# lucidrains/x-clip

Measured on AMD Instinct MI355X. Metric: image-text pairs/sec (fwd+bwd) at global batch; MFMA% + HBM GB/s, higher is better.
Workload: dtype bf16; 1 GPU; BASELINE configs[1]: default CLIP dim 512 depth 6/6 image 256 patch 32 text seq 256, patch dropout 0.5, InfoNCE, fwd+bwd; the last text layer computes only the CLS row the head reads (the same loss and gradients up to bf16 rounding order; the dense layer is timed in `dense_last_layer` with --full); workload_tag=default-infonce-b1024, local_batch=1024, global_batch=1024, parallelism=dp1, text_last_layer_rows=cls-only

## Files before the change

include/xclip.h:

```cpp
#ifndef XCLIP_H
#define XCLIP_H
#include <stdint.h>

#ifdef __cplusplus
extern "C" {
#endif

enum { XCLIP_F32 = 0, XCLIP_BF16 = 1 };
#define XCLIP_ABI_VERSION 28

int xclip_abi_version(void);
const char* xclip_last_error(void);
const char* xclip_build_info(void);
int xclip_clock_sample(uint64_t* out2, int64_t ticks_10ns, void* stream);

int xclip_layernorm_fwd(const void* x, int64_t ldx, const void* g, const void* res, void* y, int64_t ldy, int64_t y_grp,
                        float* mean, float* rstd, int64_t rows, int64_t dim, float eps, int geglu, int dtype, void* stream);
int64_t xclip_layernorm_bwd_workspace_bytes(int64_t rows, int64_t dim);
int xclip_layernorm_bwd(const void* dy, const void* x, int64_t ldx, const void* g, const float* mean, const float* rstd,
                        const void* dres, void* dx, int64_t lddx, float* dg_accum, void* workspace, int64_t workspace_bytes,
                        int64_t rows, int64_t dim, int geglu, int dtype, void* stream);

int xclip_layernorm_chain_fwd(const void* p, const void* g1, const void* res, void* x1, float* mean1, float* rstd1, const void* g2,
                              void* h2, float* mean2, float* rstd2, int64_t rows, int64_t dim, float eps, int dtype, void* stream);
int64_t xclip_layernorm_chain_bwd_workspace_bytes(int64_t rows, int64_t dim);
int xclip_layernorm_chain_bwd(const void* dh2, const void* x1, const void* g2, const float* mean2, const float* rstd2, const void* dres,
                              void* dx1, const void* p, const void* g1, const float* mean1, const float* rstd1, void* dp, float* dg2_accum,
                              float* dg1_accum, void* workspace, int64_t workspace_bytes, int64_t rows, int64_t dim, int dtype, void* stream);
int xclip_l2norm_fwd(const void* x, void* y, float* rnorm, int64_t rows, int64_t dim, int dtype, void* stream);
int xclip_l2norm_bwd(const void* dy, const void* y, const float* rnorm, void* dx, int64_t rows, int64_t dim, int dtype, void* stream);

int xclip_text_embed_fwd(const int64_t* tokens, const void* E, const void* P, const void* cls, void* out,
                         int64_t batch, int64_t n, int64_t dim, int64_t vocab, int32_t* bad_token_flag, int dtype, void* stream);
int xclip_text_embed_bwd(const void* dout, const int64_t* tokens, float* dE_accum, float* dP_accum, float* dcls_accum,
                         int64_t batch, int64_t n, int64_t dim, int64_t vocab, int has_cls, int dtype, void* stream);

int xclip_patchify(const void* image, const int32_t* keep, void* out, int64_t ldo, int64_t batch, int64_t channels,
                   int64_t height, int64_t width, int64_t patch, int64_t nkeep, int dtype, void* stream);

int xclip_token_mean_fwd(const void* x, int64_t x_batch_stride, void* out, int64_t batch, int64_t n, int64_t dim, int dtype,
                         void* stream);
int xclip_token_mean_bwd(const void* dout, const void* dsrc, int64_t src_batch_stride, void* dx, int64_t batch, int64_t n,
                         int64_t dim, int dtype, void* stream);

int xclip_copy_rows(const void* src, int64_t lds, void* dst, int64_t ldd, int64_t rows, int64_t dim, int dtype, void* stream);

int xclip_add(const void* a, const void* b, void* out, int64_t count, int dtype, void* stream);

int64_t xclip_rows_scatter_add_workspace_bytes(int64_t rows, int64_t dim);
int xclip_rows_scatter_add(const void* src, int64_t lds, const int32_t* idx, float* table_accum, float* colsum_accum,
                           int64_t rows, int64_t dim, void* workspace, int64_t workspace_bytes, int dtype, void* stream);

int xclip_scatter_add_sorted(const void* src, int64_t lds, const int64_t* sorted_ids, const int64_t* perm, float* table_accum,
                             int64_t table_rows, int64_t count, int64_t dim, int64_t n_in, int64_t n_out, int64_t row_off, int dtype,
                             void* stream);

int64_t xclip_sort_ids_workspace_bytes(int64_t count);
int xclip_sort_ids(const int64_t* ids, int64_t count, int64_t id_limit, int64_t* sorted_ids, int64_t* perm, void* workspace,
                   int64_t workspace_bytes, void* stream);

int xclip_cast_from_f32(const float* src, void* dst, int64_t count, float scale, int dtype, void* stream);

int64_t xclip_gemm_workspace_bytes(int64_t M, int64_t N, int64_t K, int dtype);
int xclip_gemm(int a_kmajor, int b_kmajor, const void* A, int64_t lda, const void* B, int64_t ldb, void* C, int64_t ldc,
               int64_t M, int64_t N, int64_t K, float alpha, const void* bias, const void* residual, int64_t ldr,
               const void* addrows, const int32_t* rowidx, int64_t ld_add, void* workspace, int64_t workspace_bytes,
               int dtype, void* stream);
int64_t xclip_gemm_small_limit(int64_t max_flop);

int xclip_gemm_batched(int a_kmajor, int b_kmajor, const void* A, int64_t lda, int64_t stride_a, const void* B, int64_t ldb, int64_t stride_b,
                       void* C, int64_t ldc, int64_t stride_c, int64_t batch, int64_t M, int64_t N, int64_t K, float alpha, int dtype,
                       void* stream);
int xclip_rowdot(const void* a, int64_t lda, const void* b, int64_t ldb, void* out, int64_t rows, int64_t dim, int dtype, void* stream);

int xclip_ffn_dgrad_geglu_ok(int64_t M, int64_t F, int64_t D, int dtype);
int64_t xclip_ffn_dgrad_geglu_workspace_bytes(int64_t M, int64_t F, int64_t D);
int xclip_ffn_dgrad_geglu(const void* dout, int64_t ldd, const void* w2, int64_t ldw, const void* x, int64_t ldx, const void* gamma,
                          const float* mean, const float* rstd, const void* x2, int64_t ld2, const void* x1, int64_t ld1, void* dx,
                          int64_t lddx, float* dg_accum, void* workspace, int64_t workspace_bytes, int64_t M, int64_t F, int64_t D,
                          int dtype, void* stream);
int xclip_ffn_wgamma(const void* w2, int64_t ldw, const void* gamma, float* wg, int64_t D, int64_t F, int dtype, void* stream);
int xclip_layernorm_bwd_ffnstats(const void* dy, const void* x, int64_t ldx, const void* g, const float* mean, const float* rstd,
                                 const void* dres, void* dx, int64_t lddx, float* dg_accum, void* workspace, int64_t workspace_bytes,
                                 int64_t rows, int64_t dim, const void* x1_below, int64_t ld1, const float* wg, const float* mean4,
                                 const float* rstd4, float inv_f, float* rowc, int dtype, void* stream);
int xclip_ffn_dgrad_geglu_rowc(const void* dout, int64_t ldd, const void* w2, int64_t ldw, const void* x, int64_t ldx, const void* gamma,
                               const float* rowc, void* dx, int64_t lddx, float* dg_accum, void* workspace, int64_t workspace_bytes,
                               int64_t M, int64_t F, int64_t D, int dtype, void* stream);

int xclip_attention_fwd(const void* qkv, const uint8_t* mask, void* out, float* lse, int64_t batch, int64_t n,
                        int64_t heads, int64_t head_dim, float scale, int causal, float dropout_p, uint64_t dropout_seed, int dtype,
                        void* stream);
int xclip_attention_bwd(const void* qkv, const uint8_t* mask, const void* out, const void* dout, const float* lse,
                        float* delta_ws, void* dqkv, int64_t batch, int64_t n, int64_t heads, int64_t head_dim, float scale, int causal,
                        float dropout_p, uint64_t dropout_seed, int dtype, void* stream);
int xclip_attention_pool_fwd(const void* q, const void* kv, const uint8_t* mask, void* out, float* lse, int64_t batch, int64_t n,
                             int64_t heads, int64_t head_dim, float scale, int64_t visible_keys, int dtype, void* stream);
int xclip_attention_pool_bwd(const void* q, const void* kv, const uint8_t* mask, const void* out, const void* dout, const float* lse,
                             void* dq, void* dkv, int64_t batch, int64_t n, int64_t heads, int64_t head_dim, float scale,
                             int64_t visible_keys, int dtype, void* stream);
int xclip_dropout(const void* x, void* y, int64_t n, float p, uint64_t seed, int dtype, void* stream);

int64_t xclip_simloss_workspace_bytes(int64_t nq, int64_t nk);
int xclip_simloss_partial(const void* Q, const void* K, int64_t nq, int64_t nk, int64_t d, float scale, const float* log_scale,
                          int64_t diag_off, int dcl, void* workspace, int64_t tile_slot0, int64_t tile_slots, float* pos,
                          int dtype, void* stream);
int xclip_simloss_combine(const void* workspace, int64_t nq, int64_t tile_slots, const float* pos, float* lse, float* loss_accum,
                          float coef, void* stream);
int xclip_simloss_fwd(const void* Q, const void* K, int64_t nq, int64_t nk, int64_t d, float scale, const float* log_scale,
                      int64_t diag_off, int dcl, float coef, void* workspace, float* pos, float* lse, float* loss_accum, int dtype,
                      void* stream);
int xclip_simloss_grad(const void* Q, const void* K, int64_t nq, int64_t nk, int64_t d, float scale, const float* log_scale,
                       int64_t diag_off, int dcl, float a, float c, float e, const float* gmul, int g_times_scale,
                       const float* lse_q, const float* lse_k, void* G, int64_t ldg, float* dtau_accum, int dtype, void* stream);

int64_t xclip_simrank_workspace_bytes(int64_t nq, int64_t nk);
int xclip_simrank_pos(const void* Q, const void* K, int64_t nq, int64_t nk, int64_t d, float scale, const float* log_scale,
                      int64_t diag_off, float* thr, int dtype, void* stream);
int xclip_simrank_partial(const void* Q, const void* K, int64_t nq, int64_t nk, int64_t d, float scale, const float* log_scale,
                          int64_t diag_off, int64_t col0, const float* thr, void* workspace, int64_t tile_slot0, int64_t tile_slots,
                          int dtype, void* stream);
int xclip_simrank_combine(const void* workspace, int64_t nq, int64_t tile_slots, int32_t* rank, float* hard_val, int32_t* hard_idx,
                          void* stream);

int64_t xclip_simtopk_workspace_bytes(int64_t nq, int64_t nk);
int xclip_simtopk_select(const void* workspace, int64_t nq, int64_t tile_slots, int64_t k, float* tau, void* stream);
int xclip_simtopk_mask(const void* Q, const void* K, int64_t nq, int64_t nk, int64_t d, float scale, const float* log_scale,
                       const float* tau, void* workspace, int64_t tile_slot0, int64_t tile_slots, int dtype, void* stream);
int xclip_simtopk_finish(const void* Q, const void* K, int64_t nq, int64_t nk, int64_t d, float scale, const float* log_scale,
                         int64_t col0, const void* workspace, int64_t tile_slot0, int64_t tile_slots, int64_t k, float* values,
                         int32_t* indices, int dtype, void* stream);

int64_t xclip_sigloss_workspace_bytes(int64_t nq, int64_t nk);
int xclip_sigloss_partial(const void* Q, const void* K, int64_t nq, int64_t nk, int64_t d, float scale, const float* log_scale,
                          const float* bias, int64_t diag_off, void* workspace, int64_t tile_slot0, int64_t tile_slots, int dtype,
                          void* stream);
int xclip_sigloss_combine(const void* workspace, int64_t nq, int64_t tile_slots, float* rowloss, float* loss_accum, float coef,
                          void* stream);
int xclip_sigloss_grad(const void* Q, const void* K, int64_t nq, int64_t nk, int64_t d, float scale, const float* log_scale,
                       const float* bias, int64_t diag_off, float coef, const float* gmul, int g_times_scale, void* G, int64_t ldg,
                       float* dtau_accum, float* dbias_accum, int dtype, void* stream);

int xclip_filip_reduce(const void* S, int64_t lds, const uint8_t* mask, const float* log_temp, float* t2i, float* i2t, int64_t ldo,
                       int16_t* kmax, int16_t* tmax, float* cnt, int64_t bx, int64_t nt, int64_t yc, int64_t ni, int64_t y0,
                       int64_t ytotal, int dtype, void* stream);
int xclip_filip_route(void* P, int64_t ldp, int64_t pcols, const uint8_t* mask, const float* log_temp, const float* g1, const float* g2, int64_t ldg,
                      const int16_t* kmax, const int16_t* tmax, const float* cnt, int64_t bx, int64_t nt, int64_t yc, int64_t ni,
                      int64_t y0, int64_t ytotal, int dtype, void* stream);
int xclip_filip_fused_ok(int64_t nt, int64_t ni, int64_t d, int dtype);
int64_t xclip_filip_fused_workspace_bytes(int64_t bx, int64_t nt, int64_t yc, int64_t ni);
int xclip_filip_fused_fwd(const void* X, const uint8_t* mask, const void* Y, const float* log_temp, float* t2i, float* i2t, int64_t ldo,
                          int16_t* kmax, int16_t* tmax, float* cnt, void* workspace, int64_t workspace_bytes, int64_t bx, int64_t nt,
                          int64_t yc, int64_t ni, int64_t d, int64_t y0, int64_t ytotal, int dtype, void* stream);
int xclip_rowlse(const float* S, int64_t lds, int64_t rows, int64_t cols, int64_t diag_off, int dcl, float coef, float* lse,
                 float* loss_accum, void* stream);
int xclip_rowgrad(const float* S, int64_t lds, const float* lse, int64_t rows, int64_t cols, int64_t diag_off, int dcl, float coef,
                  const float* gmul, float* G, int64_t ldg, float* dtau_accum, void* stream);
int xclip_gather_rows(const void* src, int64_t lds, const int32_t* idx, void* out, int64_t rows, int64_t dim, int dtype, void* stream);
int xclip_cross_entropy_fwd(const void* logits, int64_t ld, const int64_t* labels, int64_t rows, int64_t cols, float* lse, float* loss_accum,
                            int dtype, void* stream);
int xclip_cross_entropy_bwd(void* logits, int64_t ld, const int64_t* labels, const float* lse, const float* gmul, int64_t rows, int64_t cols,
                            int dtype, void* stream);
int64_t xclip_dwconv4s2_workspace_bytes(int64_t batch, int64_t h, int64_t C, int dtype);
int xclip_dwconv4s2_fwd(const void* x, const void* w, void* y, int64_t batch, int64_t h, int64_t C, int dtype, void* stream);
int xclip_dwconv4s2_bwd(const void* dy, const void* x, const void* w, void* dx, float* dw_accum, void* workspace, int64_t workspace_bytes,
                        int64_t batch, int64_t h, int64_t C, int dtype, void* stream);
int xclip_rotary(void* x, int64_t ld, int64_t rows, int64_t n, int64_t slots, int64_t slot_width, int64_t rot, const float* inv_freq, int inverse,
                 int dtype, void* stream);
int xclip_simreg_diff(const void* A, int64_t lda, const void* C, int64_t ldc, void* D, int64_t ldd, int64_t rows, int64_t cols,
                      int64_t diag_off, float* sumsq_accum, int dtype, void* stream);

int64_t xclip_batchnorm_workspace_bytes(int64_t rows, int64_t cols);
int xclip_batchnorm_fwd(const void* x, const float* gamma, const float* beta, void* y, float* mean, float* rstd, float* running_mean,
                        float* running_var, float momentum, float eps, int training, int relu, int64_t rows, int64_t cols,
                        void* workspace, int64_t workspace_bytes, int dtype, void* stream);
int xclip_batchnorm_bwd(const void* x, const void* dy, const float* gamma, const float* beta, const float* mean, const float* rstd,
                        void* dx, float* dgamma, float* dbeta, int training, int relu, int64_t rows, int64_t cols, void* workspace,
                        int64_t workspace_bytes, int dtype, void* stream);
// ... 17 lines not shown
```

x_clip_amd/_lib.py:

```python
from __future__ import annotations

import ctypes
import os
from ctypes import c_char_p, c_double, c_float, c_int, c_int64, c_uint64, c_void_p

import torch

_HERE = os.path.dirname(os.path.abspath(__file__))
LIB_PATH = os.path.join(_HERE, "libxclip_hip.so")

_lib = None
_is_emulator = False

P, I, L, F, U, D = c_void_p, c_int, c_int64, c_float, c_uint64, c_double

_SIGNATURES = {
    "xclip_abi_version": (c_int, []),
    "xclip_last_error": (c_char_p, []),
    "xclip_build_info": (c_char_p, []),
    "xclip_clock_sample": (c_int, [P, L, P]),
    "xclip_layernorm_fwd": (c_int, [P, L, P, P, P, L, L, P, P, L, L, F, I, I, P]),
    "xclip_layernorm_bwd_workspace_bytes": (c_int64, [L, L]),
    "xclip_layernorm_bwd": (c_int, [P, P, L, P, P, P, P, P, L, P, P, L, L, L, I, I, P]),
    "xclip_l2norm_fwd": (c_int, [P, P, P, L, L, I, P]),
    "xclip_l2norm_bwd": (c_int, [P, P, P, P, L, L, I, P]),
    "xclip_text_embed_fwd": (c_int, [P, P, P, P, P, L, L, L, L, P, I, P]),
    "xclip_text_embed_bwd": (c_int, [P, P, P, P, P, L, L, L, L, I, I, P]),
    "xclip_patchify": (c_int, [P, P, P, L, L, L, L, L, L, L, I, P]),
    "xclip_token_mean_fwd": (c_int, [P, L, P, L, L, L, I, P]),
    "xclip_token_mean_bwd": (c_int, [P, P, L, P, L, L, L, I, P]),
    "xclip_copy_rows": (c_int, [P, L, P, L, L, L, I, P]),
    "xclip_add": (c_int, [P, P, P, L, I, P]),
    "xclip_rows_scatter_add_workspace_bytes": (c_int64, [L, L]),
    "xclip_rows_scatter_add": (c_int, [P, L, P, P, P, L, L, P, L, I, P]),
    "xclip_scatter_add_sorted": (c_int, [P, L, P, P, P, L, L, L, L, L, L, I, P]),
    "xclip_sort_ids_workspace_bytes": (L, [L]),
    "xclip_sort_ids": (c_int, [P, L, L, P, P, P, L, P]),
    "xclip_cast_from_f32": (c_int, [P, P, L, F, I, P]),
    "xclip_gemm_workspace_bytes": (c_int64, [L, L, L, I]),
    "xclip_gemm_small_limit": (c_int64, [L]),
    "xclip_gemm": (c_int, [I, I, P, L, P, L, P, L, L, L, L, F, P, P, L, P, P, L, P, L, I, P]),
    "xclip_ffn_dgrad_geglu_ok": (c_int, [L, L, L, I]),
    "xclip_ffn_dgrad_geglu_workspace_bytes": (c_int64, [L, L, L]),
    "xclip_ffn_dgrad_geglu": (c_int, [P, L, P, L, P, L, P, P, P, P, L, P, L, P, L, P, P, L, L, L, L, I, P]),
    "xclip_ffn_wgamma": (c_int, [P, L, P, P, L, L, I, P]),
    "xclip_layernorm_bwd_ffnstats": (c_int, [P, P, L, P, P, P, P, P, L, P, P, L, L, L, P, L, P, P, P, F, P, I, P]),
    "xclip_ffn_dgrad_geglu_rowc": (c_int, [P, L, P, L, P, L, P, P, P, L, P, P, L, L, L, L, I, P]),
    "xclip_gemm_batched": (c_int, [I, I, P, L, L, P, L, L, P, L, L, L, L, L, L, F, I, P]),
    "xclip_rowdot": (c_int, [P, L, P, L, P, L, L, I, P]),
    "xclip_attention_fwd": (c_int, [P, P, P, P, L, L, L, L, F, I, F, U, I, P]),
    "xclip_attention_bwd": (c_int, [P, P, P, P, P, P, P, L, L, L, L, F, I, F, U, I, P]),
    "xclip_attention_pool_fwd": (c_int, [P, P, P, P, P, L, L, L, L, F, L, I, P]),
    "xclip_attention_pool_bwd": (c_int, [P, P, P, P, P, P, P, P, L, L, L, L, F, L, I, P]),
    "xclip_dropout": (c_int, [P, P, L, F, U, I, P]),
    "xclip_filip_reduce": (c_int, [P, L, P, P, P, P, L, P, P, P, L, L, L, L, L, L, I, P]),
    "xclip_filip_fused_ok": (c_int, [L, L, L, I]),
    "xclip_filip_fused_workspace_bytes": (c_int64, [L, L, L, L]),
    "xclip_filip_fused_fwd": (c_int, [P, P, P, P, P, P, L, P, P, P, P, L, L, L, L, L, L, L, L, I, P]),
    "xclip_filip_route": (c_int, [P, L, L, P, P, P, P, L, P, P, P, L, L, L, L, L, L, I, P]),
    "xclip_rowlse": (c_int, [P, L, L, L, L, I, F, P, P, P]),
    "xclip_rowgrad": (c_int, [P, L, P, L, L, L, I, F, P, P, L, P, P]),
    "xclip_simreg_diff": (c_int, [P, L, P, L, P, L, L, L, L, P, I, P]),
    "xclip_rotary": (c_int, [P, L, L, L, L, L, L, P, I, I, P]),
    "xclip_layernorm_chain_fwd": (c_int, [P, P, P, P, P, P, P, P, P, P, L, L, F, I, P]),
    "xclip_layernorm_chain_bwd_workspace_bytes": (c_int64, [L, L]),
    "xclip_layernorm_chain_bwd": (c_int, [P, P, P, P, P, P, P, P, P, P, P, P, P, P, P, L, L, L, I, P]),
    "xclip_gather_rows": (c_int, [P, L, P, P, L, L, I, P]),
    "xclip_cross_entropy_fwd": (c_int, [P, L, P, L, L, P, P, I, P]),
    "xclip_cross_entropy_bwd": (c_int, [P, L, P, P, P, L, L, I, P]),
    "xclip_batchnorm_workspace_bytes": (c_int64, [L, L]),
    "xclip_batchnorm_fwd": (c_int, [P, P, P, P, P, P, P, P, F, F, I, I, L, L, P, L, I, P]),
    "xclip_batchnorm_bwd": (c_int, [P, P, P, P, P, P, P, P, P, I, I, L, L, P, L, I, P]),
    "xclip_neg_cosine_fwd": (c_int, [P, P, L, L, F, P, P, P, P, I, P]),
    "xclip_neg_cosine_bwd": (c_int, [P, P, P, P, P, P, F, P, L, L, I, P]),
    "xclip_dwconv4s2_workspace_bytes": (c_int64, [L, L, L, I]),
    "xclip_dwconv4s2_fwd": (c_int, [P, P, P, L, L, L, I, P]),
    "xclip_dwconv4s2_bwd": (c_int, [P, P, P, P, P, P, L, L, L, L, I, P]),
    "xclip_simloss_workspace_bytes": (c_int64, [L, L]),
    "xclip_simloss_partial": (c_int, [P, P, L, L, L, F, P, L, I, P, L, L, P, I, P]),
    "xclip_simloss_combine": (c_int, [P, L, L, P, P, P, F, P]),
    "xclip_simloss_fwd": (c_int, [P, P, L, L, L, F, P, L, I, F, P, P, P, P, I, P]),
    "xclip_simloss_grad": (c_int, [P, P, L, L, L, F, P, L, I, F, F, F, P, I, P, P, P, L, P, I, P]),
    "xclip_simrank_workspace_bytes": (c_int64, [L, L]),
    "xclip_simrank_pos": (c_int, [P, P, L, L, L, F, P, L, P, I, P]),
    "xclip_simrank_partial": (c_int, [P, P, L, L, L, F, P, L, L, P, P, L, L, I, P]),
    "xclip_simrank_combine": (c_int, [P, L, L, P, P, P, P]),
    "xclip_simtopk_workspace_bytes": (c_int64, [L, L]),
    "xclip_simtopk_select": (c_int, [P, L, L, L, P, P]),
    "xclip_simtopk_mask": (c_int, [P, P, L, L, L, F, P, P, P, L, L, I, P]),
    "xclip_simtopk_finish": (c_int, [P, P, L, L, L, F, P, L, P, L, L, L, P, P, I, P]),
    "xclip_sigloss_workspace_bytes": (c_int64, [L, L]),
    "xclip_sigloss_partial": (c_int, [P, P, L, L, L, F, P, P, L, P, L, L, I, P]),
    "xclip_sigloss_combine": (c_int, [P, L, L, P, P, F, P]),
    "xclip_sigloss_grad": (c_int, [P, P, L, L, L, F, P, P, L, F, P, I, P, L, P, P, I, P]),
    "xclip_gradnorm_partial": (c_int, [P, L, L, I, P, P]),
    "xclip_optim_prepare": (c_int, [P, L, F, I, P, P, P, L, P]),
    "xclip_adamw_step": (c_int, [P, L, L, I, I, P, P, P, P, P, D, D, D, D, D, P]),
}
EXPORTS = tuple(_SIGNATURES)
ABI_VERSION = 28


def _bind(path: str):
    lib = ctypes.CDLL(path)
    for name, (res, args) in _SIGNATURES.items():
        fn = getattr(lib, name)
        fn.restype = res
        fn.argtypes = args
    if lib.xclip_abi_version() != ABI_VERSION:
        raise RuntimeError(f"{path}: ABI version {lib.xclip_abi_version()} != {ABI_VERSION} -- rebuild (python -m x_clip_amd.build)")
    return lib


def lib():
    global _lib
    if _lib is None:
        if not os.path.exists(LIB_PATH):
            raise RuntimeError(
                f"x_clip_amd: {LIB_PATH} is missing -- build the gfx950 kernel library first "
                f"(`python -m x_clip_amd.build`). There is no CPU/PyTorch fallback.")
        _lib = _bind(LIB_PATH)
    return _lib


def is_emulator() -> bool:
    return _is_emulator


def _use_library_for_tests(path):
    global _lib, _is_emulator
    if path is None:
        _lib, _is_emulator = None, False
    else:
        _lib, _is_emulator = _bind(path), True


def use_measurement_build():
    global _lib, _is_emulator
    path = os.path.join(_HERE, "libxclip_hip_measure.so")
    if not os.path.exists(path):
        raise RuntimeError(f"{path} is missing: python -m x_clip_amd.build --measure")
    _lib, _is_emulator = _bind(path), False


def check(code: int, what: str):
    if code != 0:
        raise RuntimeError(f"{what} failed ({code}): {lib().xclip_last_error().decode()}")
```

x_clip_amd/csrc/kernels/attention.h:

```cpp
#pragma once
#include "common.h"

namespace xc {

constexpr int ATT_DH = 64;
constexpr float ATT_NEG = -3.0e38f;

struct AttnParams {
    const void* qkv;
    const unsigned char* mask;
    void* out;
    float* lse;
    const void* dout;
    float* delta;
    void* dqkv;
    int batch, n, heads;
    float scale;
    int chunks;
    int causal;
    int stagger_10ns;
    int first_round;
    uint32_t drop_thresh;
    float drop_scale;
    uint64_t drop_seed;
};

template <typename T>
struct AttCfg {
    static constexpr int VEC = Elem<T>::VEC;
    static constexpr int KB = 2 * VEC;
    static constexpr int DKB = ATT_DH / KB;
    static constexpr int NKB = 32 / KB;
    static constexpr int LD = 64 + VEC;
    static constexpr int TILE = 64 * LD;
    static constexpr int CH = 64 / VEC;
};

template <typename T, int NT>
XC_DEV void stage_rows(T* tile, const T* X, long ldx, int r0, int nrows, int tid) {
    typedef AttCfg<T> C;
    for (int u = tid; u < 64 * C::CH; u += NT) {
        const int row = u / C::CH, c = u % C::CH;
        st16(tile + row * C::LD + c * C::VEC, (r0 + row < nrows) ? ld16(X + (long)(r0 + row) * ldx + c * C::VEC) : zero16());
    }
}
template <typename T, int NT>
XC_DEV void stage_rows_transposed(T* tile, const T* X, long ldx, int r0, int nrows, int tid) {
    typedef AttCfg<T> C;
    for (int u = tid; u < 16 * C::CH; u += NT) {
        const int rg = u / C::CH, c = u % C::CH;
        u32x4 r[4];
#pragma unroll
        for (int i = 0; i < 4; ++i) {
            const int row = r0 + rg * 4 + i;
            r[i] = (row < nrows) ? ld16(X + (long)row * ldx + c * C::VEC) : zero16();
        }
        tr4_store(tile, C::LD, c * C::VEC, rg * 4, r);
    }
}

XC_DEV u32x4 frag_from_acc(const f32x16& acc, int blk, bf16_t*) {
    u32x4 f;
#pragma unroll
    for (int w = 0; w < 4; ++w)
        f[w] = f2bf_pk(acc[8 * blk + 2 * w], acc[8 * blk + 2 * w + 1]);
    return f;
}
XC_DEV u32x4 frag_from_acc(const f32x16& acc, int blk, float*) {
    u32x4 f = {f2u(acc[4 * blk]), f2u(acc[4 * blk + 1]), f2u(acc[4 * blk + 2]), f2u(acc[4 * blk + 3])};
    return f;
}
XC_DEV u32x4 load_tr_frag(const bf16_t* rowp, int base, int blk, int h) {
    const u32x2 lo = *reinterpret_cast<const u32x2*>(rowp + base + 16 * blk + 4 * h);
    const u32x2 hi = *reinterpret_cast<const u32x2*>(rowp + base + 16 * blk + 4 * h + 8);
    u32x4 f = {lo[0], lo[1], hi[0], hi[1]};
    return f;
}
XC_DEV u32x4 load_tr_frag(const float* rowp, int base, int blk, int h) { return ld16(rowp + base + 8 * blk + 4 * h); }

template <typename T, int NW>
XC_DEV void store_rows_via_lds(T* Os, const f32x16 (&acc)[2], float mul, T* dst, long ldd, int row0, int nrows, int lane,
                               int wave) {
    typedef AttCfg<T> C;
    const int c31 = lane & 31;
#pragma unroll
    for (int db = 0; db < 2; ++db)
#pragma unroll
        for (int r = 0; r < 16; ++r)
            Os[(wave * 32 + c31) * C::LD + db * 32 + mfma_row(r, lane)] = from_f32<T>(acc[db][r] * mul);
    sync();
    for (int u = lane; u < 32 * C::CH; u += 64) {
        const int row = u / C::CH, c = u % C::CH;
        if (row0 + row < nrows) st16(dst + (long)(row0 + row) * ldd + c * C::VEC, ld16(Os + (wave * 32 + row) * C::LD + c * C::VEC));
    }
    sync();
}

template <typename T, int NW, int NH = 1>
__global__ __launch_bounds__(NW * 64) void attn_fwd_kernel(AttnParams p) {
    typedef AttCfg<T> C;
    constexpr int NT = NW * 64;
    constexpr int DH = ATT_DH * NH;
    XC_LDS_DYNAMIC(lds);
    T* Ks = reinterpret_cast<T*>(lds);
    T* Vt = Ks + NH * C::TILE;
    T* Os = Vt + NH * C::TILE;
    unsigned char* Ms = reinterpret_cast<unsigned char*>(Os + NW * 32 * C::LD);
// ... 342 lines not shown
```

x_clip_amd/csrc/kernels/attention3.h:

```cpp
#pragma once
#include "attention2.h"

namespace xc {

constexpr int A3_MAX_N = 288;

XC_DEV void a3_dma_image(unsigned char* img, const bf16_t* X, long ldx, int n, int npad, int wave, int nwaves, int lane) {
    const int pieces = npad >> 3;
    for (int pc = wave; pc < pieces; pc += nwaves) {
        const int row = pc * 8 + (lane >> 3);
        const int chunk = a2_slot(row, lane & 7);
        const int g = row < n ? row : n - 1;
        glds16(X + (long)g * ldx + chunk * 8, img + pc * 1024);
    }
}

constexpr int A3_TAIL_MAX = 2;
XC_HOST_DEV bool a3_coop_tail(int n) { return (n & 31) != 0 && (n & 31) <= A3_TAIL_MAX && n >= 64; }
XC_HOST_DEV int a3_waves(int n) { return a3_coop_tail(n) ? n / 32 : (n + 31) / 32; }
constexpr int A3_TAIL_REC = 66;

XC_DEV u32x4 a3_row_frag(const unsigned char* img, int t, int kb, int lane) {
    const int c31 = lane & 31, h = lane >> 5;
    return ld16(img + t * 4096 + (c31 * 128 + a2_slot(c31, kb * 2 + h) * 16));
// ... 332 lines not shown
            dk[db] = mma_kblock(a3_col_frag(Qs, t, blk, db, lane), df, dk[db], (bf16_t*)nullptr);
        }
    }
}
template <bool CAUSAL>
XC_DEV void a3_bwd_dkv_sweep(const unsigned char* Qs, const unsigned char* dOs, const float* Ls2, const float* Ds, int t0, int tend, int dt,
                             int n, bool keys_plain, const u32x4 (&kf)[4], const u32x4 (&vf)[4], bool kvalid, float scale2, int lane,
                             int kidx, f32x16 (&dk)[2], f32x16 (&dv)[2]) {
    for (int t = t0; t < tend; t += dt) {
        u32x4 qa[4], da[4];
        a3_tile_rows(Qs, t, lane, qa);
        a3_tile_rows(dOs, t, lane, da);
        a3_bwd_dkv_step<CAUSAL>(Qs, dOs, Ls2, Ds, t, n, qa, da, kf, vf, kvalid, scale2, lane, kidx, dk, dv, !(keys_plain && t * 32 + 32 <= n));
    }
}
XC_DEV void a3_put_col(float* rec, const f32x16 (&acc)[2], int lane) {
#pragma unroll
    for (int db = 0; db < 2; ++db)
#pragma unroll
        for (int r = 0; r < 16; ++r) rec[db * 32 + mfma_row(r, lane)] = acc[db][r];
}

XC_DEV void a3_store_rows_direct(const f32x16 (&acc)[2], bf16_t* dst, long ldd, int row0, int nrows, int lane, float mul = 1.f) {
    const int c31 = lane & 31, h = lane >> 5;
    const int row = row0 + c31;
#pragma unroll
    for (int db = 0; db < 2; ++db) {
        uint32_t pk[4][2];
#pragma unroll
        for (int q = 0; q < 4; ++q) {
            pk[q][0] = f2bf_pk(acc[db][4 * q] * mul, acc[db][4 * q + 1] * mul);
            pk[q][1] = f2bf_pk(acc[db][4 * q + 2] * mul, acc[db][4 * q + 3] * mul);
        }
#pragma unroll
        for (int qq = 0; qq < 4; qq += 2) {
            permlane32_swap(pk[qq][0], pk[qq + 1][0]);
            permlane32_swap(pk[qq][1], pk[qq + 1][1]);
            if (row < nrows) {
                u32x4 o = {pk[qq][0], pk[qq][1], pk[qq + 1][0], pk[qq + 1][1]};
                st16(dst + (long)row * ldd + db * 32 + qq * 8 + 8 * h, o);
            }
        }
    }
}
XC_DEV void a3_row_frags(const bf16_t* X, long ldx, int r, int lane, u32x4 (&f)[4]) {
    const int h = lane >> 5;
#pragma unroll
    for (int kb = 0; kb < 4; ++kb) f[kb] = ld16(X + (long)r * ldx + kb * 16 + h * 8);
}

template <bool CAUSAL>
__global__ __launch_bounds__(256) void attn3_bwd_kernel(AttnParams p) {
    XC_LDS_DYNAMIC(lds);
    const int n = p.n, npad = (n + 31) & ~31;
    const int img = npad * 128;
    unsigned char* R0 = lds;
    unsigned char* R1 = R0 + img;
    unsigned char* Ms = R1 + img;
    float* Ls = reinterpret_cast<float*>(Ms + npad);
    float* Ds = Ls + npad;
    float* Tp = Ds + npad;
    const int tid = threadIdx.x, lane = tid & 63, h = lane >> 5, c31 = lane & 31;
    const int wave = uniform(tid >> 6), nwaves = blockDim.x >> 6;
    a3_stagger(p.stagger_10ns, p.first_round);
    const int bh = xcd_remap(blockIdx.x, p.batch * p.heads);
    const int hh = bh % p.heads, bi = bh / p.heads;
    const long ldq = 3L * p.heads * ATT_DH, ldo = (long)p.heads * ATT_DH;
    const bf16_t* Qb = reinterpret_cast<const bf16_t*>(p.qkv) + (long)bi * n * ldq + hh * ATT_DH;
    const bf16_t* Kb = Qb + (long)p.heads * ATT_DH;
    const bf16_t* Vb = Kb + (long)p.heads * ATT_DH;
    const bf16_t* dOb = reinterpret_cast<const bf16_t*>(p.dout) + (long)bi * n * ldo + hh * ATT_DH;
    const bf16_t* Ob = reinterpret_cast<const bf16_t*>(p.out) + (long)bi * n * ldo + hh * ATT_DH;
    bf16_t* dQ = reinterpret_cast<bf16_t*>(p.dqkv) + (long)bi * n * ldq + hh * ATT_DH;
    bf16_t* dK = dQ + (long)p.heads * ATT_DH;
    bf16_t* dV = dK + (long)p.heads * ATT_DH;
    a3_dma_image(R0, Kb, ldq, n, npad, wave, nwaves, lane);
    a3_dma_image(R1, Vb, ldq, n, npad, wave, nwaves, lane);
    a3_key_validity(Ms, p.mask, (long)bi * n, n, npad);
    const bool coop = a3_coop_tail(n);
    const int tail0 = (n >> 5) << 5, ntail = n & 31;
    const int nblk = a3_waves(n);
    const int nsub = npad >> 5;
    const float scale2 = p.scale * 1.4426950408889634f;
    for (int blk = wave; blk < nsub; blk += nwaves) {
        const int row_ = blk * 32 + c31;
        const int rl = row_ < n ? row_ : n - 1;
        const float lse_r = p.lse[((long)bi * p.heads + hh) * n + rl];
        float acc = 0.f;
#pragma unroll
        for (int c = 0; c < 4; ++c) {
            float a[8], b[8];
            load_vec<bf16_t>(Ob + (long)rl * ldo + h * 32 + c * 8, a);
            load_vec<bf16_t>(dOb + (long)rl * ldo + h * 32 + c * 8, b);
#pragma unroll
            for (int k = 0; k < 8; ++k) acc += a[k] * b[k];
        }
        acc += shfl_xor(acc, 32);
        if (h == 0) {
            Ds[row_] = row_ < n ? acc : 0.f;
            Ls[row_] = row_ < n ? lse_r * 1.4426950408889634f : 0.f;
        }
    }
    wait_vmem();
    sync();
    uint32_t plain_bits = 0;
    for (int t = 0; t < nsub; ++t) plain_bits |= wave_all(Ms[t * 32 + c31] != 0) ? (1u << t) : 0u;

    u32x4 f0[4], f1[4];
    f32x16 g0[2], g1[2];
    if (!(p.chunks & 1)) {
        if (coop) {
            const int trow = tail0 + c31 < n ? tail0 + c31 : n - 1;
            a3_row_frags(Qb, ldq, trow, lane, f0);
            a3_row_frags(dOb, ldo, trow, lane, f1);
#pragma unroll
            for (int db = 0; db < 2; ++db)
#pragma unroll
                for (int r = 0; r < 16; ++r) g0[db][r] = 0.f;
            const float lq = Ls[tail0 + c31], dl = Ds[tail0 + c31];
            int tcoop = nsub;
            if (a3_single_tail(n, p.chunks)) {
                tcoop = nsub - 1;
                const float st = a3_tail_dot(R0, tcoop, 0, f0, lane), dt_ = a3_tail_dot(R1, tcoop, 0, f1, lane);
                if (wave == nwaves - 1 && Ms[tail0] != 0) a3_tail_outer(R0, tcoop, 0, fast_exp2(st * scale2 - lq) * (dt_ - dl), lane, g0);
            }
            a3_bwd_dq_sweep<CAUSAL>(R0, R1, Ms, wave, tcoop, nwaves, plain_bits, f0, f1, lq, dl, scale2, lane, tail0 + c31, g0);
            if (c31 < ntail) a3_put_col(Tp + ((long)wave * A3_TAIL_MAX + c31) * 128, g0, lane);
        }
        for (int rb = wave; rb < nblk; rb += nwaves) {
            const int row = rb * 32 + c31;
            const int rl = row < n ? row : n - 1;
            a3_row_frags(Qb, ldq, rl, lane, f0);
            a3_row_frags(dOb, ldo, rl, lane, f1);
#pragma unroll
            for (int db = 0; db < 2; ++db)
#pragma unroll
                for (int r = 0; r < 16; ++r) g0[db][r] = 0.f;
            const float lse_q = Ls[row], delta_q = Ds[row];
            int tend = CAUSAL ? (rb + 1 < nsub ? rb + 1 : nsub) : nsub;
            if (a3_single_tail(n, p.chunks) && !CAUSAL) {
                tend = nsub - 1;
                if (Ms[tail0] != 0) {
                    const float pt = fast_exp2(a3_tail_dot(R0, tend, 0, f0, lane) * scale2 - lse_q);
                    const float ds = pt * (a3_tail_dot(R1, tend, 0, f1, lane) - delta_q);
                    a3_tail_outer(R0, tend, 0, ds, lane, g0);
                }
            }
            a3_bwd_dq_sweep<CAUSAL>(R0, R1, Ms, 0, tend, 1, plain_bits, f0, f1, lse_q, delta_q, scale2, lane, row, g0);
            a3_store_rows_direct(g0, dQ, ldq, rb * 32, n, lane, p.scale);
        }
    }
    sync();
    a3_dma_image(R0, Qb, ldq, n, npad, wave, nwaves, lane);
    a3_dma_image(R1, dOb, ldo, n, npad, wave, nwaves, lane);
    if (coop && wave == 0 && !(p.chunks & 1)) {
        for (int q = 0; q < ntail; ++q) {
            float acc = 0.f;
            for (int w = 0; w < nwaves; ++w) acc += Tp[((long)w * A3_TAIL_MAX + q) * 128 + lane];
            dQ[(long)(tail0 + q) * ldq + lane] = f2bf(acc * p.scale);
        }
    }
    wait_vmem();
    sync();

    if (!(p.chunks & 2)) {
        for (int rb = wave; rb < nblk; rb += nwaves) {
            const int row = rb * 32 + c31;
            const int rl = row < n ? row : n - 1;
            a3_row_frags(Kb, ldq, rl, lane, f0);
            a3_row_frags(Vb, ldq, rl, lane, f1);
            const bool kvalid = Ms[row] != 0;
#pragma unroll
            for (int db = 0; db < 2; ++db)
#pragma unroll
                for (int r = 0; r < 16; ++r) { g0[db][r] = 0.f; g1[db][r] = 0.f; }
            const bool keys_plain = wave_all(kvalid);
            int qend = nsub;
            if (a3_single_tail(n, p.chunks)) {
                qend = nsub - 1;
                const float st = a3_tail_dot(R0, qend, 0, f0, lane);
// ... 68 lines not shown
```

x_clip_amd/csrc/kernels/attention5.h:

```cpp
#pragma once
#include "attention3.h"

namespace xc {

constexpr int A5_MIN_BLOCKS = 7;
constexpr int A5_TILE = 32 * 64;

XC_DEV void a5_tile_put(unsigned char* tile, int c31, int h, int g, u32x2 v) {
    *reinterpret_cast<u32x2*>(tile + c31 * 64 + ((g ^ ((c31 >> 2) & 3)) << 4) + 8 * h) = v;
}
XC_DEV u32x4 a5_tile_frag(const unsigned char* tile, int blk, int lane) {
    const int g = lane >> 4, tt = lane & 15;
    const int r0 = 16 * blk + 4 * (g >> 1) + (tt >> 2);
    const int col = 16 * (g & 1) + (tt & 3) * 4;
    const int lo_off = r0 * 64 + (((col >> 3) ^ ((r0 >> 2) & 3)) << 4) + (col & 7) * 2;
    const int hi_off = (r0 + 8) * 64 + (((col >> 3) ^ (((r0 + 8) >> 2) & 3)) << 4) + (col & 7) * 2;
    const s16x4 lo = lds_read_tr16(tile + lo_off);
    const s16x4 hi = lds_read_tr16(tile + hi_off);
    const u32x2 a = __builtin_bit_cast(u32x2, lo), b = __builtin_bit_cast(u32x2, hi);
    u32x4 f = {a[0], a[1], b[0], b[1]};
    return f;
}

XC_HOST_DEV bool a5_takes(int n, int causal) { return !causal && ((n & 31) == 0 || (n & 31) == 1) && (n >> 5) >= 2 && (n >> 5) <= 8; }
// ... 62 lines not shown
    }
#pragma unroll
    for (int hf = 0; hf < 2; ++hf) {
        wave_sync();
        if ((c31 >> 4) == hf) {
#pragma unroll
            for (int db = 0; db < 2; ++db)
#pragma unroll
                for (int q2 = 0; q2 < 2; ++q2) {
                    const int j = 4 * db + 2 * q2 + h;
                    *reinterpret_cast<u32x4*>(tile + r16 * 128 + ((j ^ (r16 & 7)) << 4)) = ch[db][q2];
                }
        }
        wave_sync();
#pragma unroll
        for (int jr = 0; jr < 2; ++jr) {
            const int r = (lane >> 3) + 8 * jr, j = lane & 7;
            const u32x4 v = *reinterpret_cast<const u32x4*>(tile + r * 128 + ((j ^ (r & 7)) << 4));
            const int row = row0 + 16 * hf + r;
            if (row < nrows) st16(dst + (long)row * ldd + j * 8, v);
        }
    }
}

__global__ __launch_bounds__(512) void attn5_bwd_kernel(AttnParams p) {
    XC_LDS_DYNAMIC(lds);
    const int n = p.n, nb = n >> 5, tail = n & 31, npad = (n + 31) & ~31, nsub = npad >> 5;
    const int img = npad * 128;
    unsigned char* Qs = lds;
    unsigned char* dOs = Qs + img;
    unsigned char* Ks = dOs + img;
    unsigned char* Xs = Ks + img;
    unsigned char* Ms = Xs + 2 * nb * A5_TILE;
    float* Ls = reinterpret_cast<float*>(Ms + npad);
    float* Ds = Ls + npad;
    float* Tp = Ds + npad;
    float* Sc = Tp + nb * 192;
    const int tid = threadIdx.x, lane = tid & 63, h = lane >> 5, c31 = lane & 31;
    const int wave = uniform(tid >> 6), nwaves = nb;
    const int bh = xcd_remap(blockIdx.x, p.batch * p.heads);
    const int hh = bh % p.heads, bi = bh / p.heads;
    const long ldq = 3L * p.heads * ATT_DH, ldo = (long)p.heads * ATT_DH;
    const float scale2 = p.scale * 1.4426950408889634f;
    const int row = wave * 32 + c31;
    const bf16_t* Qb = reinterpret_cast<const bf16_t*>(p.qkv) + (long)bi * n * ldq + hh * ATT_DH;
    const bf16_t* Kb = Qb + (long)p.heads * ATT_DH;
    const bf16_t* Vb = Kb + (long)p.heads * ATT_DH;
    const bf16_t* dOb = reinterpret_cast<const bf16_t*>(p.dout) + (long)bi * n * ldo + hh * ATT_DH;
    const bf16_t* Ob = reinterpret_cast<const bf16_t*>(p.out) + (long)bi * n * ldo + hh * ATT_DH;
    bf16_t* dQ = reinterpret_cast<bf16_t*>(p.dqkv) + (long)bi * n * ldq + hh * ATT_DH;
    bf16_t* dK = dQ + (long)p.heads * ATT_DH;
    bf16_t* dV = dK + (long)p.heads * ATT_DH;
    const float* const lse_h = p.lse + ((long)bi * p.heads + hh) * n;
#ifdef XCLIP_MEASURE
    const int var = uniform(p.chunks);
#else
    constexpr int var = 0;
#endif
    auto delta_of = [&](int row_, const u32x4 (&a)[4], const u32x4 (&b)[4], float lse_r) {
        float acc = 0.f;
#pragma unroll
        for (int c = 0; c < 4; ++c) {
            float fa[8], fb[8];
            unpack(a[c], fa, (bf16_t*)nullptr);
            unpack(b[c], fb, (bf16_t*)nullptr);
#pragma unroll
            for (int k = 0; k < 8; ++k) acc += fa[k] * fb[k];
        }
        acc += shfl_xor(acc, 32);
        if (h == 0) {
            Ds[row_] = row_ < n ? acc : 0.f;
            Ls[row_] = row_ < n ? lse_r * 1.4426950408889634f : 0.f;
        }
    };
    auto delta_rows = [&](int row_, u32x4 (&a)[4], u32x4 (&b)[4]) {
        const int rl = row_ < n ? row_ : n - 1;
#pragma unroll
        for (int c = 0; c < 4; ++c) {
            a[c] = ld16(Ob + (long)rl * ldo + h * 32 + c * 8);
            b[c] = ld16(dOb + (long)rl * ldo + h * 32 + c * 8);
        }
        return lse_h[rl];
    };
    {
        u32x4 a[4], b[4];
        float lse_r = 0.f;
        if (!(var & 2)) lse_r = delta_rows(row, a, b);
        a3_dma_image(Qs, Qb, ldq, n, npad, wave, nwaves, lane);
        a3_dma_image(dOs, dOb, ldo, n, npad, wave, nwaves, lane);
        a3_dma_image(Ks, Kb, ldq, n, npad, wave, nwaves, lane);
        a3_key_validity(Ms, p.mask, (long)bi * n, n, npad);
        if (var & 2) lse_r = delta_rows(row, a, b);
        delta_of(row, a, b, lse_r);
        for (int blk = wave + nwaves; blk < nsub; blk += nwaves) {
            const float lse_t = delta_rows(blk * 32 + c31, a, b);
            delta_of(blk * 32 + c31, a, b, lse_t);
        }
    }
    u32x4 kf[4], vf[4];
    a3_row_frags(Kb, ldq, row, lane, kf);
    a3_row_frags(Vb, ldq, row, lane, vf);
    wait_vmem();
    sync();
    const bool kvalid = Ms[row] != 0;
    const bool masked = !wave_all(kvalid);
    f32x16 dk[2], dv[2], dq[2];
#pragma unroll
    for (int db = 0; db < 2; ++db)
#pragma unroll
        for (int r = 0; r < 16; ++r) { dk[db][r] = 0.f; dv[db][r] = 0.f; dq[db][r] = 0.f; }
    float* const sc = Sc + wave * 64;
    if (tail) {
        const int trow = 32 * nb;
        {
            const float st = a3_tail_dot(Qs, nb, 0, kf, lane), dpt = a3_tail_dot(dOs, nb, 0, vf, lane);
            const float pt = kvalid ? fast_exp2(st * scale2 - Ls[trow]) : 0.f;
            const float ds = pt * (dpt - Ds[trow]);
            a3_tail_outer(Qs, nb, 0, ds, lane, dk);
            a3_tail_outer(dOs, nb, 0, pt, lane, dv);
            a5_weighted_row_sum(Ks, wave, sc, ds, lane, Tp + (wave * 3 + 0) * 64);
        }
        {
            u32x4 qf[4], dof[4];
            a3_row_frags(Qb, ldq, row, lane, qf);
            a3_row_frags(dOb, ldo, row, lane, dof);
            const float st = a3_tail_dot(Ks, nb, 0, qf, lane), dpt = a5_row_dot(Vb + (long)trow * ldq, dof, lane);
            const float pt = Ms[trow] != 0 ? fast_exp2(st * scale2 - Ls[row]) : 0.f;
            const float ds = pt * (dpt - Ds[row]);
            a3_tail_outer(Ks, nb, 0, ds, lane, dq);
            a5_weighted_row_sum(Qs, wave, sc, ds, lane, Tp + (wave * 3 + 1) * 64);
            a5_weighted_row_sum(dOs, wave, sc, pt, lane, Tp + (wave * 3 + 2) * 64);
        }
    }
    auto produce = [&](int s) {
        const int t = wave + s < nb ? wave + s : wave + s - nb;
        unsigned char* const myX = Xs + ((s & 1) * nb + wave) * A5_TILE;
        u32x4 qa[4], da[4];
        a3_tile_rows(Qs, t, lane, qa);
        a3_tile_rows(dOs, t, lane, da);
        f32x16 sv, dp;
        float l2[16], dl[16];
#pragma unroll
        for (int q = 0; q < 4; ++q) {
            const u32x4 a = ld16(Ls + t * 32 + 8 * q + 4 * h), b = ld16(Ds + t * 32 + 8 * q + 4 * h);
#pragma unroll
            for (int e = 0; e < 4; ++e) { l2[4 * q + e] = u2f(a[e]); dl[4 * q + e] = u2f(b[e]); }
        }
#pragma unroll
        for (int r = 0; r < 16; ++r) { sv[r] = 0.f; dp[r] = -dl[r]; }
#pragma unroll
        for (int kb = 0; kb < 4; ++kb) {
            sv = mma_kblock(qa[kb], kf[kb], sv, (bf16_t*)nullptr);
            dp = mma_kblock(da[kb], vf[kb], dp, (bf16_t*)nullptr);
        }
        if (masked) {
#pragma unroll
            for (int r = 0; r < 16; ++r) {
                const float pv = kvalid ? fast_exp2(sv[r] * scale2 - l2[r]) : 0.f;
                sv[r] = pv;
                dp[r] = pv * dp[r];
            }
        } else {
#pragma unroll
            for (int r = 0; r < 16; ++r) {
                sv[r] = fast_exp2(sv[r] * scale2 - l2[r]);
                dp[r] = sv[r] * dp[r];
            }
// ... 66 lines not shown
```

x_clip_amd/csrc/kernels/gemm2.h:

```cpp
#pragma once
#include "gemm.h"

namespace xc {

constexpr int G2_BM = 256, G2_BN = 256, G2_BK = 64, G2_THREADS = 512;
constexpr int G2_OPER_BYTES = 256 * 64 * 2;
constexpr int G2_STAGE_BYTES = 2 * G2_OPER_BYTES;
constexpr int G2_LDC = 256 + 4;
constexpr int G2_LDS_BYTES = 2 * G2_STAGE_BYTES;

template <bool KMAJOR>
XC_DEV void g2_stage(const bf16_t* X, long ld, int outer0, int nouter, int k0, unsigned char* tile, int wave, int lane) {
#pragma unroll
    for (int q = 0; q < 4; ++q) {
        const int id = wave * 4 + q;
        const bf16_t* src;
        if (!KMAJOR) {
            const int row = id * 8 + (lane >> 3);
            const int chunk = (lane & 7) ^ ((row >> 1) & 7);
            int g = outer0 + row;
            g = g < nouter ? g : nouter - 1;
            src = X + (long)g * ld + k0 + chunk * 8;
        } else {
            const int panel = id >> 3;
            const int row = (id & 7) * 8 + (lane >> 3);
            const int chunk = (lane & 7) ^ (((row >> 1) & 1) << 2);
            int g = outer0 + panel * 64 + chunk * 8;
            g = g < nouter ? g : nouter - 8;
            src = X + (long)(k0 + row) * ld + g;
        }
        glds16(src, tile + id * 1024);
    }
}

template <bool KMAJOR>
XC_DEV void g2_stage_piece(const bf16_t* X, long ld, int outer0, int nouter, int k0, unsigned char* tile, int wave, int lane, int q) {
    const int id = wave * 4 + q;
    const bf16_t* src;
    if (!KMAJOR) {
        const int row = id * 8 + (lane >> 3);
        const int chunk = (lane & 7) ^ ((row >> 1) & 7);
        int g = outer0 + row;
        g = g < nouter ? g : nouter - 1;
        src = X + (long)g * ld + k0 + chunk * 8;
    } else {
        const int panel = id >> 3;
        const int row = (id & 7) * 8 + (lane >> 3);
        const int chunk = (lane & 7) ^ (((row >> 1) & 1) << 2);
        int g = outer0 + panel * 64 + chunk * 8;
        g = g < nouter ? g : nouter - 8;
        src = X + (long)(k0 + row) * ld + g;
    }
    glds16(src, tile + id * 1024);
}

XC_DEV u32x4 g2_frag_normal(const unsigned char* tile, int r0, int kk, int lane) {
    const int row = r0 + (lane & 31);
    const int chunk = (kk * 2 + (lane >> 5)) ^ ((row >> 1) & 7);
    return ld16(tile + row * 128 + chunk * 16);
}
XC_DEV u32x4 g2_frag_kmajor(const unsigned char* tile, int c0, int kk, int lane) {
    const int g = lane >> 4, tt = lane & 15;
    const int col = c0 + 16 * (g & 1) + (tt & 3) * 4;
    const int krow = kk * 16 + 8 * (g >> 1) + (tt >> 2);
    const int panel = col >> 6, colp = col & 63;
    const int chunk = (colp >> 3) ^ (((krow >> 1) & 1) << 2);
    const unsigned char* p = tile + panel * 8192 + krow * 128 + chunk * 16 + (colp & 7) * 2;
    const s16x4 lo = lds_read_tr16(p);
    const s16x4 hi = lds_read_tr16(p + 4 * 128);
    u32x2 a = __builtin_bit_cast(u32x2, lo), b = __builtin_bit_cast(u32x2, hi);
    u32x4 f = {a[0], a[1], b[0], b[1]};
    return f;
}

struct Gemm2Params {
    const bf16_t* A; const bf16_t* B; bf16_t* C;
    long lda, ldb, ldc;
    int M, N, K;
    float alpha;
    const bf16_t* bias; const bf16_t* residual; long ldr;
    const bf16_t* addrows; const int* rowidx; long ld_add;
    float* partial;
    int k_per_split;
    int tiles_m, tiles_n;
    int band_n;
    int stream_out;
    int split_lin = 0;
};

XC_DEV void g2_pair(const Gemm2Params& p, int ntiles, int& tile, int& slice, bool& valid) {
    const int total = ntiles * p.split_lin, chunk = (total + 7) >> 3;
    const int lin = blockIdx.x, j = lin >> 3, w = (lin & 7) * chunk + j;
    valid = j < chunk && w < total;
    slice = w / ntiles;
    tile = w - slice * ntiles;
}
XC_DEV bool g2_where(const Gemm2Params& p, int ntiles, int& tile0, int& slice, int& stride) {
    if (p.split_lin > 0) {
        bool valid;
        g2_pair(p, ntiles, tile0, slice, valid);
        stride = ntiles;
        return valid;
    }
    tile0 = blockIdx.x;
    slice = blockIdx.y;
    stride = gridDim.x;
    return (int)blockIdx.x < ntiles;
}
XC_DEV int g2_slice(const Gemm2Params& p, int ntiles) {
    if (p.split_lin > 0) {
        int tile, slice;
        bool valid;
        g2_pair(p, ntiles, tile, slice, valid);
        return slice;
    }
    return (int)blockIdx.y;
}

template <bool A_KMAJOR, bool B_KMAJOR>
__global__ __launch_bounds__(G2_THREADS, 2) void gemm2_kernel(Gemm2Params p) {
    XC_LDS_DYNAMIC(lds);
    const int tid = threadIdx.x;
    const int lane = tid & 63;
    const int wave = uniform(tid >> 6);
    const int wm = wave >> 2, wn = wave & 3;
    const int tile = xcd_remap(blockIdx.x, p.tiles_m * p.tiles_n);
    const int m0 = (tile / p.tiles_n) * G2_BM, n0 = (tile % p.tiles_n) * G2_BN;
    const int kbeg = blockIdx.y * p.k_per_split;
    const int kend = (kbeg + p.k_per_split < p.K) ? kbeg + p.k_per_split : p.K;
    const int nt = (kend - kbeg) / G2_BK;

    f32x16 acc[4][2];
#pragma unroll
    for (int i = 0; i < 4; ++i)
#pragma unroll
        for (int j = 0; j < 2; ++j)
#pragma unroll
            for (int r = 0; r < 16; ++r) acc[i][j][r] = 0.f;

    auto stage = [&](int buf, int k0) {
        unsigned char* base = lds + buf * G2_STAGE_BYTES;
        g2_stage<A_KMAJOR>(p.A, p.lda, m0, p.M, k0, base, wave, lane);
        g2_stage<B_KMAJOR>(p.B, p.ldb, n0, p.N, k0, base + G2_OPER_BYTES, wave, lane);
    };

    if (nt > 0) stage(0, kbeg);
    wait_vmem();
    sync();
    for (int t = 0; t < nt; ++t) {
        const unsigned char* As = lds + (t & 1) * G2_STAGE_BYTES;
        const unsigned char* Bs = As + G2_OPER_BYTES;
        if (t + 1 < nt) stage((t + 1) & 1, kbeg + (t + 1) * G2_BK);
#pragma unroll
        for (int kk = 0; kk < 4; ++kk) {
            u32x4 a[4], b[2];
#pragma unroll
            for (int i = 0; i < 4; ++i)
                a[i] = A_KMAJOR ? g2_frag_kmajor(As, wm * 128 + i * 32, kk, lane) : g2_frag_normal(As, wm * 128 + i * 32, kk, lane);
#pragma unroll
            for (int j = 0; j < 2; ++j)
                b[j] = B_KMAJOR ? g2_frag_kmajor(Bs, wn * 64 + j * 32, kk, lane) : g2_frag_normal(Bs, wn * 64 + j * 32, kk, lane);
#pragma unroll
            for (int i = 0; i < 4; ++i)
#pragma unroll
                for (int j = 0; j < 2; ++j) acc[i][j] = mma_kblock(a[i], b[j], acc[i][j], (bf16_t*)nullptr);
        }
        wait_vmem();
        sync();
    }

// ... 56 lines not shown
```

x_clip_amd/csrc/kernels/gemm4.h:

```cpp
#pragma once
#include <type_traits>
#include "gemm3.h"

namespace xc {

enum : int {
    G4_PLAIN = 0,
    G4_SLAB = 1,
    G4_TERMS = 2,
    G4_RES = 3
};

template <bool KMAJOR>
XC_DEV uint32_t g4_voff(long ld, int wave, int lane, int q) {
    const int id = wave * 4 + q;
    if (!KMAJOR) {
        const int row = id * 8 + (lane >> 3);
        const int chunk = (lane & 7) ^ ((row >> 1) & 7);
        return ((uint32_t)row * (uint32_t)ld + (uint32_t)chunk * 8u) * 2u;
    } else {
        const int panel = id >> 3;
        const int row = (id & 7) * 8 + (lane >> 3);
        const int chunk = (lane & 7) ^ (((row >> 1) & 1) << 2);
        return ((uint32_t)row * (uint32_t)ld + (uint32_t)(panel * 64 + chunk * 8)) * 2u;
    }
}
template <bool KMAJOR>
struct G4Operand {
    const bf16_t* pos;
    uint32_t bytes;
    XC_DEV void tile(const bf16_t* X, long ld, int outer0, int nouter, int k0) {
        int valid = nouter - outer0;
        valid = valid < 256 ? valid : 256;
        if (!KMAJOR) {
            pos = X + (long)outer0 * ld + k0;
            bytes = (uint32_t)(valid - 1) * (uint32_t)ld * 2u + 128u;
        } else {
            pos = X + (long)k0 * ld + outer0;
            bytes = 63u * (uint32_t)ld * 2u + (uint32_t)valid * 2u;
        }
    }
    XC_DEV void advance(long ld) { pos += KMAJOR ? (long)G2_BK * ld : (long)G2_BK; }
    XC_DEV BufRsrc rsrc() const { return make_rsrc(pos, bytes); }
};

struct G4Dma {
    BufRsrc a, b;
};

template <bool A_KMAJOR, bool B_KMAJOR, class Epilogue>
XC_DEV void g4_run(const Gemm2Params& p, unsigned char* lds, Epilogue epi) {
    const int tid = threadIdx.x;
    const int lane = tid & 63;
    const int wave = uniform(tid >> 6);
    const int wm = wave >> 2, wn = wave & 3;
    const int ntiles = p.tiles_m * p.tiles_n;
    int tile0, slice, stride;
    const bool mine = g2_where(p, ntiles, tile0, slice, stride);
    const int kbeg = slice * p.k_per_split;
    const int kend = (kbeg + p.k_per_split < p.K) ? kbeg + p.k_per_split : p.K;
    const int nt = (kend - kbeg) / G2_BK;
    if (!mine || nt <= 0) return;

    auto tile_origin = [&](int id, int& m0, int& n0) {
        const int tile = p.split_lin > 0 ? id : xcd_remap(id, ntiles);
        m0 = (tile / p.tiles_n) * G2_BM;
        n0 = (tile % p.tiles_n) * G2_BN;
    };
    const uint32_t va[2] = {g4_voff<A_KMAJOR>(p.lda, wave, lane, 0), g4_voff<A_KMAJOR>(p.lda, wave, lane, 1)};
    const uint32_t vb[2] = {g4_voff<B_KMAJOR>(p.ldb, wave, lane, 0), g4_voff<B_KMAJOR>(p.ldb, wave, lane, 1)};
    const uint32_t sa = (uint32_t)p.lda * 32u, sb = (uint32_t)p.ldb * 32u;
    unsigned char* const my0 = lds + wave * 4096;

    int did = tile0, dt = 0, dm = 0, dn = 0;
    tile_origin(did, dm, dn);
    G4Operand<A_KMAJOR> oa;
    G4Operand<B_KMAJOR> ob;
    oa.tile(p.A, p.lda, dm, p.M, kbeg);
    ob.tile(p.B, p.ldb, dn, p.N, kbeg);
    G4Dma d;
    auto dma_next = [&]() {
        if (++dt == nt) {
            if (did + stride < ntiles) {
                dt = 0;
                did += stride;
                tile_origin(did, dm, dn);
                oa.tile(p.A, p.lda, dm, p.M, kbeg);
                ob.tile(p.B, p.ldb, dn, p.N, kbeg);
            } else {
                dt = nt - 1;
            }
        } else {
            oa.advance(p.lda);
// ... 428 lines not shown
    XC_DEV bool packs_lines(int m0, int n0) const { return MODE == G4_PLAIN && (m0 + G2_BM <= p.M) && (n0 + G2_BN <= p.N); }
    XC_DEV void pack_lines(f32x16 (&acc)[4][2], unsigned char* scratch, u32x4 (&o)[4][4], int = 0, int = 0) const {
        if (p.alpha == 1.f) pack_lines_t<true>(acc, scratch, o);
        else pack_lines_t<false>(acc, scratch, o);
    }
    template <bool NT = false>
    XC_DEV void store_lines(const u32x4 (&o)[4][4], int m0, int n0) const {
        const int lane = threadIdx.x & 63;
        const int wave = uniform(threadIdx.x >> 6), wm = wave >> 2, wn = wave & 3;
        const BufRsrc rc = make_rsrc(p.C + (long)m0 * p.ldc + n0, 255u * (uint32_t)p.ldc * 2u + 512u);
        const uint32_t vc = ((uint32_t)(wm * 128 + (lane >> 3)) * (uint32_t)p.ldc + (uint32_t)(wn * 64 + 8 * (lane & 7))) * 2u;
        const uint32_t s8 = (uint32_t)p.ldc * 16u;
#pragma unroll
        for (int i = 0; i < 4; ++i)
#pragma unroll
            for (int k = 0; k < 4; ++k) {
                if (NT) buf_st16_nt<0>(rc, vc, s8 * (uint32_t)(4 * i + k), o[i][k]);
                else buf_st16<0>(rc, vc, s8 * (uint32_t)(4 * i + k), o[i][k]);
            }
    }
    template <bool NT, int NG>
    XC_DEV void store_line_groups(const u32x4 (&o)[NG][4], int i0, int m0, int n0) const {
        const int lane = threadIdx.x & 63;
        const int wave = uniform(threadIdx.x >> 6), wm = wave >> 2, wn = wave & 3;
        const BufRsrc rc = make_rsrc(p.C + (long)m0 * p.ldc + n0, 255u * (uint32_t)p.ldc * 2u + 512u);
        const uint32_t vc = ((uint32_t)(wm * 128 + (lane >> 3)) * (uint32_t)p.ldc + (uint32_t)(wn * 64 + 8 * (lane & 7))) * 2u;
        const uint32_t s8 = (uint32_t)p.ldc * 16u;
#pragma unroll
        for (int i = 0; i < NG; ++i)
#pragma unroll
            for (int k = 0; k < 4; ++k) {
                if (NT) buf_st16_nt<0>(rc, vc, s8 * (uint32_t)(4 * (i0 + i) + k), o[i][k]);
                else buf_st16<0>(rc, vc, s8 * (uint32_t)(4 * (i0 + i) + k), o[i][k]);
            }
    }
    template <bool NT = false>
    XC_DEV void store_full_res_lds(f32x16 (&acc)[4][2], int m0, int n0, unsigned char* scratch) const {
        const int lane = threadIdx.x & 63, r = lane & 31, h = lane >> 5;
        const int wave = uniform(threadIdx.x >> 6), wm = wave >> 2, wn = wave & 3;
        const BufRsrc rc = make_rsrc(p.C + (long)m0 * p.ldc + n0, 255u * (uint32_t)p.ldc * 2u + 512u);
        const BufRsrc rr = make_rsrc(p.residual + (long)m0 * p.ldr + n0, 255u * (uint32_t)p.ldr * 2u + 512u);
        const uint32_t vc = ((uint32_t)(wm * 128 + (lane >> 3)) * (uint32_t)p.ldc + (uint32_t)(wn * 64 + 8 * (lane & 7))) * 2u;
        const uint32_t vr = ((uint32_t)(wm * 128 + (lane >> 3)) * (uint32_t)p.ldr + (uint32_t)(wn * 64 + 8 * (lane & 7))) * 2u;
        const uint32_t c8 = (uint32_t)p.ldc * 16u, r8 = (uint32_t)p.ldr * 16u;
        unsigned char* const quad = scratch + r * 128 + 8 * h;
        unsigned char* const line = scratch + (lane >> 3) * 128 + (((lane & 7) ^ (lane >> 3)) << 4);
        const float al = p.alpha;
        u32x4 res[2][4];
#pragma unroll
        for (int k = 0; k < 4; ++k) res[0][k] = buf_ld16<0>(rr, vr, r8 * (uint32_t)k);
#pragma unroll
        for (int i = 0; i < 4; ++i) {
            if (i < 3) {
#pragma unroll
                for (int k = 0; k < 4; ++k) res[(i + 1) & 1][k] = buf_ld16<0>(rr, vr, r8 * (uint32_t)(4 * (i + 1) + k));
            }
#pragma unroll
            for (int k = 0; k < 4; ++k) *reinterpret_cast<u32x4*>(line + k * 1024) = res[i & 1][k];
            lds_fence();
#pragma unroll
            for (int j = 0; j < 2; ++j) {
#pragma unroll
                for (int q = 0; q < 4; ++q) {
                    unsigned char* const at = quad + (((4 * j + q) ^ (r & 7)) << 4);
                    const u32x2 rv = *reinterpret_cast<const u32x2*>(at);
                    const float* a = reinterpret_cast<const float*>(&acc[i][j]) + 4 * q;
                    const u32x2 v = {f2bf_pk(a[0] * al + u2f(rv[0] << 16), a[1] * al + u2f(rv[0] & 0xffff0000u)),
                                     f2bf_pk(a[2] * al + u2f(rv[1] << 16), a[3] * al + u2f(rv[1] & 0xffff0000u))};
                    *reinterpret_cast<u32x2*>(at) = v;
                }
            }
            lds_fence();
            u32x4 o[4];
#pragma unroll
            for (int k = 0; k < 4; ++k) o[k] = *reinterpret_cast<const u32x4*>(line + k * 1024);
            lds_fence();
#pragma unroll
            for (int k = 0; k < 4; ++k) {
                if (NT) buf_st16_nt<0>(rc, vc, c8 * (uint32_t)(4 * i + k), o[k]);
                else buf_st16<0>(rc, vc, c8 * (uint32_t)(4 * i + k), o[k]);
            }
        }
    }
    XC_DEV void store_full_slab_lds(f32x16 (&acc)[4][2], int m0, int n0, unsigned char* scratch) const {
        const int lane = threadIdx.x & 63, r = lane & 31, h = lane >> 5;
        const int wave = uniform(threadIdx.x >> 6), wm = wave >> 2, wn = wave & 3;
        const float* slab = p.partial + ((long)g2_slice(p, p.tiles_m * p.tiles_n) * p.M + m0) * p.N + n0;
        const BufRsrc rc = make_rsrc(slab, 255u * (uint32_t)p.N * 4u + 1024u);
        const uint32_t vc = ((uint32_t)(wm * 128 + (lane >> 3)) * (uint32_t)p.N + (uint32_t)(wn * 64 + 4 * (lane & 7))) * 4u;
        const uint32_t s8 = (uint32_t)p.N * 32u;
        unsigned char* const wr = scratch + r * 128;
        const unsigned char* const rd = scratch + (lane >> 3) * 128 + (((lane & 7) ^ (lane >> 3)) << 4);
#pragma unroll
        for (int i = 0; i < 4; ++i) {
#pragma unroll
            for (int j = 0; j < 2; ++j) {
#pragma unroll
                for (int q = 0; q < 4; ++q) {
                    const u32x4 v = {f2u(acc[i][j][4 * q]), f2u(acc[i][j][4 * q + 1]), f2u(acc[i][j][4 * q + 2]), f2u(acc[i][j][4 * q + 3])};
                    *reinterpret_cast<u32x4*>(wr + (((2 * q + h) ^ (r & 7)) << 4)) = v;
                }
                lds_fence();
                u32x4 o[4];
#pragma unroll
                for (int k = 0; k < 4; ++k) o[k] = *reinterpret_cast<const u32x4*>(rd + k * 1024);
                lds_fence();
#pragma unroll
                for (int k = 0; k < 4; ++k) {
                    if (j == 0) buf_st16<0>(rc, vc, s8 * (uint32_t)(4 * i + k), o[k]);
                    else buf_st16<128>(rc, vc, s8 * (uint32_t)(4 * i + k), o[k]);
                }
            }
        }
    }
    XC_DEV int with_scratch(f32x16 (&acc)[4][2], int m0, int n0, unsigned char* scratch) const {
        const bool full = (m0 + G2_BM <= p.M) && (n0 + G2_BN <= p.N);
        if (MODE == G4_SLAB && full) {
            store_full_slab_lds(acc, m0, n0, scratch);
            return 32;
        }
        if (MODE == G4_RES && full) {
            store_full_res_lds<false>(acc, m0, n0, scratch);
            return 0;
        }
        return (*this)(acc, m0, n0);
    }

    XC_DEV int operator()(f32x16 (&acc)[4][2], int m0, int n0) const {
        const bool full = (m0 + G2_BM <= p.M) && (n0 + G2_BN <= p.N);
        if (MODE == G4_PLAIN) {
            if (full) { store_bf16<true>(acc, m0, n0); return 16; }
            store_bf16<false>(acc, m0, n0);
            return 0;
        }
        (void)G3GemmEpilogue<0>{p}(acc, m0, n0);
        return 0;
    }
};

struct G4ProbeEpilogue {
    const Gemm2Params& p;
    XC_DEV void finish() const {}
    XC_DEV int operator()(f32x16 (&acc)[4][2], int m0, int n0) const {
        const int lane = threadIdx.x & 63;
        const int wave = uniform(threadIdx.x >> 6), wm = wave >> 2, wn = wave & 3;
        const BufRsrc rc = make_rsrc(p.C + (long)m0 * p.ldc + n0, 255u * (uint32_t)p.ldc * 2u + 512u);
        const uint32_t vc = ((uint32_t)(wm * 128 + (lane >> 3)) * (uint32_t)p.ldc + (uint32_t)(wn * 64 + 8 * (lane & 7))) * 2u;
        const uint32_t s8 = (uint32_t)p.ldc * 16u;
#pragma unroll
        for (int i = 0; i < 4; ++i) {
#pragma unroll
            for (int j = 0; j < 2; ++j) {
                uint32_t pk[4][2];
#pragma unroll
                for (int q = 0; q < 4; ++q) {
                    pk[q][0] = f2bf_pk(acc[i][j][4 * q] * p.alpha, acc[i][j][4 * q + 1] * p.alpha);
                    pk[q][1] = f2bf_pk(acc[i][j][4 * q + 2] * p.alpha, acc[i][j][4 * q + 3] * p.alpha);
                }
                permlane32_swap(pk[0][0], pk[1][0]);
                permlane32_swap(pk[0][1], pk[1][1]);
                permlane32_swap(pk[2][0], pk[3][0]);
                permlane32_swap(pk[2][1], pk[3][1]);
                const u32x4 o0 = {pk[0][0], pk[0][1], pk[1][0], pk[1][1]};
                const u32x4 o1 = {pk[2][0], pk[2][1], pk[3][0], pk[3][1]};
                buf_st16<0>(rc, vc, s8 * (uint32_t)(4 * i + 2 * j), o0);
                buf_st16<0>(rc, vc, s8 * (uint32_t)(4 * i + 2 * j + 1), o1);
            }
        }
        return 16;
    }
    XC_DEV bool packs_lines(int, int) const { return false; }
    XC_DEV int with_scratch(f32x16 (&acc)[4][2], int m0, int n0, unsigned char*) const { return (*this)(acc, m0, n0); }
    XC_DEV void pack_lines(f32x16 (&)[4][2], unsigned char*, u32x4 (&)[4][4], int = 0, int = 0) const {}
    template <bool NT = false> XC_DEV void store_lines(const u32x4 (&)[4][4], int, int) const {}
    template <bool NT, int NG> XC_DEV void store_line_groups(const u32x4 (&)[NG][4], int, int, int) const {}
};

template <bool A_KMAJOR, bool B_KMAJOR, int MODE, int ABL = 0>
__global__ __launch_bounds__(G2_THREADS, 2) void gemm5_kernel(Gemm2Params p) {
    XC_LDS_DYNAMIC(lds);
    if constexpr ((ABL & 64) != 0) g5_run<A_KMAJOR, B_KMAJOR, G4ProbeEpilogue, ABL>(p, lds, G4ProbeEpilogue{p});
    else g5_run<A_KMAJOR, B_KMAJOR, G4GemmEpilogue<MODE>, ABL>(p, lds, G4GemmEpilogue<MODE>{p});
}

template <bool A_KMAJOR, bool B_KMAJOR, int MODE>
__global__ __launch_bounds__(G2_THREADS, 2) void gemm4_kernel(Gemm2Params p) {
    XC_LDS_DYNAMIC(lds);
    g4_run<A_KMAJOR, B_KMAJOR>(p, lds, G4GemmEpilogue<MODE>{p});
}

}
```

x_clip_amd/csrc/kernels/rows.h:

```cpp
#pragma once
#include "common.h"

namespace xc {

template <typename T, int MAXC, bool GEGLU, bool NT = false>
XC_DEV void load_row(const T* xr, int D, int lane, float (&v)[MAXC][Elem<T>::VEC]) {
    constexpr int VEC = Elem<T>::VEC;
    const int nch = D / VEC;
#pragma unroll
    for (int i = 0; i < MAXC; ++i) {
        const int c = lane + 64 * i;
        if (c < nch) {
            load_vec<T, NT>(xr + c * VEC, v[i]);
            if (GEGLU) {
                float gt[VEC];
                load_vec<T, NT>(xr + D + c * VEC, gt);
#pragma unroll
                for (int j = 0; j < VEC; ++j) v[i][j] *= gelu_erf(gt[j]);
            }
        } else {
#pragma unroll
            for (int j = 0; j < VEC; ++j) v[i][j] = 0.f;
        }
    }
// ... 571 lines not shown

template <typename T, int MAXC>
__global__ __launch_bounds__(256) void l2norm_fwd_kernel(const T* __restrict__ x, T* __restrict__ y,
                                                         float* __restrict__ rnorm_out, int rows, int D) {
    constexpr int VEC = Elem<T>::VEC;
    const int lane = lane_id();
    const long row = (long)blockIdx.x * 4 + wave_id();
    if (row >= rows) return;
    const int nch = D / VEC;
    float v[MAXC][VEC];
    load_row<T, MAXC, false>(x + row * (long)D, D, lane, v);
    float q = 0.f;
#pragma unroll
    for (int i = 0; i < MAXC; ++i)
#pragma unroll
        for (int j = 0; j < VEC; ++j) q += v[i][j] * v[i][j];
    const float nrm = sqrtf(wave_sum(q));
    const float rn = 1.0f / fmaxf(nrm, 1e-12f);
#pragma unroll
    for (int i = 0; i < MAXC; ++i) {
        const int c = lane + 64 * i;
        if (c < nch) {
            float o[VEC];
#pragma unroll
            for (int j = 0; j < VEC; ++j) o[j] = v[i][j] * rn;
            store_vec<T>(y + row * (long)D + c * VEC, o);
        }
    }
    if (lane == 0) rnorm_out[row] = rn;
}

template <typename T, int MAXC>
__global__ __launch_bounds__(256) void rowdot_kernel(const T* __restrict__ a, long lda, const T* __restrict__ b, long ldb, T* __restrict__ out,
                                                     int rows, int D) {
    constexpr int VEC = Elem<T>::VEC;
    const int lane = lane_id();
    const long row = (long)blockIdx.x * 4 + wave_id();
    if (row >= rows) return;
    float u[MAXC][VEC], w[MAXC][VEC];
    load_row<T, MAXC, false>(a + row * lda, D, lane, u);
    load_row<T, MAXC, false>(b + row * ldb, D, lane, w);
    const int nch = D / VEC;
    float q = 0.f;
#pragma unroll
    for (int i = 0; i < MAXC; ++i)
        if (lane + 64 * i < nch)
#pragma unroll
            for (int j = 0; j < VEC; ++j) q += u[i][j] * w[i][j];
    q = wave_sum(q);
    if (lane == 0) out[row] = from_f32<T>(q);
}

template <typename T, int MAXC>
__global__ __launch_bounds__(256) void l2norm_bwd_kernel(const T* __restrict__ dy, const T* __restrict__ y,
                                                         const float* __restrict__ rnorm, T* __restrict__ dx,
                                                         int rows, int D) {
    constexpr int VEC = Elem<T>::VEC;
    const int lane = lane_id();
    const long row = (long)blockIdx.x * 4 + wave_id();
    if (row >= rows) return;
    const int nch = D / VEC;
    float yv[MAXC][VEC], dv[MAXC][VEC];
    load_row<T, MAXC, false>(y + row * (long)D, D, lane, yv);
    load_row<T, MAXC, false>(dy + row * (long)D, D, lane, dv);
    float dot = 0.f;
#pragma unroll
    for (int i = 0; i < MAXC; ++i)
#pragma unroll
        for (int j = 0; j < VEC; ++j) dot += yv[i][j] * dv[i][j];
    dot = wave_sum(dot);
    const float rn = rnorm[row];
#pragma unroll
    for (int i = 0; i < MAXC; ++i) {
        const int c = lane + 64 * i;
        if (c < nch) {
            float o[VEC];
#pragma unroll
            for (int j = 0; j < VEC; ++j) o[j] = (dv[i][j] - yv[i][j] * dot) * rn;
            store_vec<T>(dx + row * (long)D + c * VEC, o);
        }
    }
}

}
```

x_clip_amd/csrc/xclip_api.hip:

```cpp
#include "xc_device.h"

#include "api_common.h"
#include "kernels/colnorm.h"
#include "kernels/filip.h"
#include "kernels/filip5.h"
#include "kernels/gemm.h"
#include "kernels/gemm2.h"
#include "kernels/gemm3.h"
#include "kernels/gemm4.h"
#include "kernels/gemm8.h"
#include "kernels/gemm9.h"
#include "kernels/gemm_small.h"
#include "kernels/optim.h"
#ifdef XCLIP_MEASURE
#include "kernels/measure/gemm6.h"
#include "kernels/measure/gemm7.h"
#endif
#include "kernels/rows.h"
#include "kernels/simloss.h"
#include "kernels/simloss5.h"
#include "kernels/simrank.h"
#include "kernels/simtopk.h"
#include "kernels/sigloss.h"
#include "kernels/sort.h"
// ... 927 lines not shown
    if (max_flop >= 0) g_small_flop = max_flop;
    return was;
}
static int gemm_small_run(const GemmArgs& g, hipStream_t st) {
    GemmSmallParams q;
    q.A = (const bf16_t*)g.A; q.B = (const bf16_t*)g.B; q.C = (bf16_t*)g.C; q.lda = g.lda; q.ldb = g.ldb; q.ldc = g.ldc;
    q.M = (int)g.M; q.N = (int)g.N; q.K = (int)g.K; q.alpha = g.alpha; q.residual = (const bf16_t*)g.residual; q.ldr = g.ldr;
    q.tiles_m = (int)(g.M / GS_BM); q.tiles_n = (int)(g.N / GS_BN);
    const int64_t tiles = (int64_t)q.tiles_m * q.tiles_n;
    q.stages = gs_stages(tiles, g.K / GS_BK);
    const int lds = q.stages * GS_STAGE_BYTES;
#define XC_GS(RES) do { XC_ALLOW_LDS((gemm_small_kernel<AK, BK_, RES>), GS_MAX_STAGES * GS_STAGE_BYTES); \
        hipLaunchKernelGGL((gemm_small_kernel<AK, BK_, RES>), dim3((unsigned)tiles), dim3(GS_THREADS), lds, st, q); } while (0)
    by_layout(g.a_kmajor, g.b_kmajor, [&](auto ak, auto bk) {
        constexpr bool AK = decltype(ak)::value, BK_ = decltype(bk)::value;
        if (g.residual != nullptr) XC_GS(true); else XC_GS(false);
    });
#undef XC_GS
    return check_launch(__func__);
}


#ifdef XCLIP_MEASURE
extern "C" int xclip_measure_gemm8(int on) { const int was = gemm8_on() ? 1 : 0; g_gemm8 = on; return was; }
#endif

int64_t xclip_gemm_workspace_bytes(int64_t M, int64_t N, int64_t K, int dtype) {
    GemmArgs g{}; g.M = M; g.N = N; g.K = K;
    return gemm_plan(g, dtype, INT64_MAX, -1).workspace_bytes;
}

int xclip_gemm(int a_kmajor, int b_kmajor, const void* A, int64_t lda, const void* B, int64_t ldb, void* C, int64_t ldc,
               int64_t M, int64_t N, int64_t K, float alpha, const void* bias, const void* residual, int64_t ldr,
               const void* addrows, const int32_t* rowidx, int64_t ld_add, void* workspace, int64_t workspace_bytes,
               int dtype, void* stream) {
    XC_REQUIRE(dtype_ok(dtype), "bad dtype");
    const int vec = vec_of(dtype);
    XC_REQUIRE(M >= 0 && N > 0 && K > 0, "bad shape");
    XC_REQUIRE(N % vec == 0 && ldc % vec == 0, "N and ldc must be multiples of the 16-byte chunk");
    XC_REQUIRE(lda % vec == 0 && ldb % vec == 0, "lda / ldb must be multiples of the 16-byte chunk");
    const int64_t Kp = (K + vec - 1) / vec * vec, Mp = (M + vec - 1) / vec * vec;
    XC_REQUIRE(a_kmajor ? (lda >= Mp) : (lda >= Kp), "lda must cover A's contiguous dim rounded up to the 16-byte chunk");
    XC_REQUIRE(b_kmajor ? (ldb >= N) : (ldb >= Kp), "ldb must cover B's contiguous dim rounded up to the 16-byte chunk");
    XC_REQUIRE(!(a_kmajor && !b_kmajor), "layout (A k-major, B normal) is not used on this path");
    XC_REQUIRE(aligned16(A) && aligned16(B) && aligned16(C) && aligned16(bias) && aligned16(residual) && aligned16(addrows) && aligned16(workspace),
               "pointers must be 16-byte aligned");
    XC_REQUIRE(residual == nullptr || ldr % vec == 0, "ldr must be a multiple of the 16-byte chunk");
    XC_REQUIRE(addrows == nullptr || (rowidx != nullptr && ld_add % vec == 0), "addrows needs rowidx and an aligned ld");
    if (M == 0) return 0;
    hipStream_t st = (hipStream_t)stream;
    const GemmArgs g{a_kmajor, b_kmajor, A, lda, B, ldb, C, ldc, M, N, K, alpha, bias, residual, ldr, addrows, rowidx, ld_add, workspace, workspace_bytes};
    const GemmPlan plan = gemm_plan(g, dtype, workspace != nullptr ? workspace_bytes : 0, g_small_flop);
    switch (plan.route) {
    case GEMM_SMALL: return gemm_small_run(g, st);
    case GEMM_256: return gemm2_run(g, plan.splits, plan.k_per_split, true, st);
    case GEMM_256_CUT: {
        GemmArgs main = g, tail = g;
        main.M = plan.main_rows;
        if (const int rc = gemm2_run(main, 1, (int)K, true, st)) return rc;
        tail.M = plan.tail_rows;
        tail.A = (const char*)A + plan.main_rows * lda * 2;
        tail.C = (char*)C + plan.main_rows * ldc * 2;
        tail.residual = nullptr; tail.ldr = 0;
        if (const int rc = gemm2_run(tail, plan.splits, plan.k_per_split, false, st)) return rc;
        const char* Rt = residual != nullptr ? (const char*)residual + plan.main_rows * ldr * 2 : nullptr;
        launch_splitk_reduce<bf16_t>(workspace, tail.C, ldc, tail.M, N, plan.splits, alpha, Rt, ldr, st);
        return check_launch(__func__);
    }
    case GEMM_GENERIC: break;
    }
    GemmParams p;
    p.A = A; p.B = B; p.C = C; p.lda = lda; p.ldb = ldb; p.ldc = ldc;
    p.M = (int)M; p.N = (int)N; p.K = (int)K; p.alpha = alpha;
    p.bias = bias; p.residual = residual; p.ldr = ldr; p.addrows = addrows; p.rowidx = rowidx; p.ld_add = ld_add;
    p.tiles_m = (int)((M + 127) / 128); p.tiles_n = (int)((N + 127) / 128);
    p.k_per_split = plan.k_per_split;
    p.partial = plan.splits > 1 ? (float*)workspace : nullptr;
    launch_gemm(p, dtype, a_kmajor, b_kmajor, plan.splits, 1, st);
    if (plan.splits > 1)
        by_dtype(dtype, [&](auto t) { launch_splitk_reduce<typename decltype(t)::type>(workspace, C, ldc, M, N, plan.splits, alpha, nullptr, 0, st); });
    return check_launch(__func__);
}

int xclip_ffn_dgrad_geglu_ok(int64_t M, int64_t F, int64_t D, int dtype) {
    return dtype == XCLIP_BF16 && M > 0 && M % G2_BM == 0 && F % G2_BN == 0 && D % G2_BK == 0 && D >= 2 * G2_BK && D <= 4096 && F < (1L << 20) &&
           (M / G2_BM) * (F / G2_BN) < (1L << 30);
}
int64_t xclip_ffn_dgrad_geglu_workspace_bytes(int64_t M, int64_t F, int64_t D) {
    return ((D + 3) / 4 * 4 + 4 * M + 2 * (M / G2_BM) * F) * 4;
}
struct FfnDgradArgs {
    const void* dout; int64_t ldd; const void* w2; int64_t ldw; const void* x; int64_t ldx; const void* gamma;
    const float* mean; const float* rstd; const void* x2; int64_t ld2; const void* x1; int64_t ld1; const float* rowc_in;
    void* dx; int64_t lddx; float* dg_accum; void* workspace; int64_t workspace_bytes; int64_t M, F, D; int dtype; void* stream;
};
static int ffn_dgrad_geglu_run(const char* fn, const FfnDgradArgs& a) {
#define XC_REQ(cond, msg) do { if (!(cond)) return xcapi::fail(fn, msg); } while (0)
    XC_REQ(xclip_ffn_dgrad_geglu_ok(a.M, a.F, a.D, a.dtype), "shape / dtype not taken by the fused kernel (xclip_ffn_dgrad_geglu_ok)");
    XC_REQ(a.dout && a.w2 && a.x && a.gamma && a.dx && a.dg_accum, "null pointer");
    XC_REQ(a.rowc_in != nullptr || (a.mean && a.rstd && a.x2 && a.x1), "null pointer");
    XC_REQ(aligned16(a.dout) && aligned16(a.w2) && aligned16(a.x) && aligned16(a.gamma) && aligned16(a.x2) && aligned16(a.x1) && aligned16(a.dx) && aligned16(a.workspace) && aligned16(a.rowc_in),
           "pointers must be 16-byte aligned");
    XC_REQ(a.ldd % 8 == 0 && a.ldw % 8 == 0 && a.ldx % 8 == 0 && a.ld2 % 8 == 0 && a.ld1 % 8 == 0 && a.lddx % 8 == 0, "leading dimensions must be multiples of the 16-byte chunk");
    XC_REQ(a.ldd >= a.D && (a.rowc_in != nullptr || (a.ld2 >= a.D && a.ld1 >= a.D)) && a.ldw >= a.F && a.ldx >= 2 * a.F && a.lddx >= 2 * a.F, "leading dimension too small");
    XC_REQ(a.ldd < (1L << 22) && a.ldw < (1L << 22) && a.ldx < (1L << 22) && a.lddx < (1L << 22), "leading dimensions beyond the 32-bit tile offsets");
    XC_REQ(a.workspace != nullptr && a.workspace_bytes >= xclip_ffn_dgrad_geglu_workspace_bytes(a.M, a.F, a.D), "workspace too small");
#undef XC_REQ
    hipStream_t st = (hipStream_t)a.stream;
    float* wg = (float*)a.workspace;
    float* rowc = wg + (a.D + 3) / 4 * 4;
    float* slab = rowc + 4 * a.M;
    if (a.rowc_in == nullptr) {
        hipLaunchKernelGGL(ffn_wgamma_kernel, dim3((unsigned)((a.D + 3) / 4)), dim3(256), 0, st, (const bf16_t*)a.w2, (long)a.ldw, (const bf16_t*)a.gamma, wg, (int)a.D, (int)a.F);
        hipLaunchKernelGGL(ffn_rowstats_kernel, dim3((unsigned)((a.M + 3) / 4)), dim3(256), 0, st, (const bf16_t*)a.dout, (long)a.ldd, (const bf16_t*)a.x2, (long)a.ld2,
                           (const bf16_t*)a.x1, (long)a.ld1, (const float*)wg, a.mean, a.rstd, rowc, (int)a.M, (int)a.D, 1.0f / (float)a.F);
    } else {
        rowc = const_cast<float*>(a.rowc_in);
    }
    Gemm2Params q{};
    q.A = (const bf16_t*)a.dout; q.B = (const bf16_t*)a.w2; q.C = nullptr; q.lda = a.ldd; q.ldb = a.ldw; q.ldc = a.F;
    q.M = (int)a.M; q.N = (int)a.F; q.K = (int)a.D; q.alpha = 1.f;
    q.bias = nullptr; q.residual = nullptr; q.ldr = 0; q.addrows = nullptr; q.rowidx = nullptr; q.ld_add = 0; q.partial = nullptr;
    q.k_per_split = (int)a.D;
    q.tiles_m = (int)(a.M / G2_BM); q.tiles_n = (int)(a.F / G2_BN);
    q.band_n = 0;
    if (q.tiles_n > 8)
        for (int b = 8; b >= 4 && q.band_n == 0; --b)
            if (q.tiles_n % b == 0) q.band_n = b;
    q.stream_out = 1;
    GegluBwdArgs e;
    e.x = (const bf16_t*)a.x; e.ldx = a.ldx; e.dx = (bf16_t*)a.dx; e.lddx = a.lddx; e.gamma = (const bf16_t*)a.gamma;
    e.rowc = rowc; e.dg_partial = slab; e.F = (int)a.F;

    int gx = q.tiles_m * q.tiles_n;
    const int cus = xc_num_cus();
    if (gx > cus) gx = cus;
    {
#define XC_G9(N) do { XC_ALLOW_LDS(gemm9_geglu_bwd_kernel<N>, G5_LDS_BYTES); \
        hipLaunchKernelGGL(gemm9_geglu_bwd_kernel<N>, dim3((unsigned)gx, 1), dim3(G2_THREADS), G5_LDS_BYTES, st, q, e); } while (0)
#ifdef XCLIP_MEASURE
    static const int abl = measure_env("XCLIP_GEMM9_ABL", 0);
    switch (abl) {
        case 1: XC_G9(1); break;
        case 2: XC_G9(2); break;
        case 4: XC_G9(4); break;
        case 8: XC_G9(8); break;
        case 14: XC_G9(14); break;
        default: XC_G9(0); break;
    }
#else
    XC_G9(0);
#endif
#undef XC_G9
    }
    const int nrows = 2 * q.tiles_m;
    int slices = nrows / 64;
    if (slices < 1) slices = 1;
    hipLaunchKernelGGL(colsum_fold_kernel, dim3((unsigned)((a.F + 63) / 64), (unsigned)slices), dim3(256), 1024, st, (const float*)slab, (long)a.F, a.dg_accum,
                       nrows, (int)a.F);
    return check_launch(fn);
}
int xclip_ffn_dgrad_geglu(const void* dout, int64_t ldd, const void* w2, int64_t ldw, const void* x, int64_t ldx, const void* gamma,
                          const float* mean, const float* rstd, const void* x2, int64_t ld2, const void* x1, int64_t ld1, void* dx,
                          int64_t lddx, float* dg_accum, void* workspace, int64_t workspace_bytes, int64_t M, int64_t F, int64_t D,
                          int dtype, void* stream) {
    XC_REQUIRE(mean && rstd && x2 && x1, "null pointer");
// ... 622 lines not shown
```

x_clip_amd/csrc/xclip_attn.hip:

```cpp
#include "xc_device.h"

#include "api_common.h"
#include "kernels/attention.h"
#include "kernels/attention2.h"
#include "kernels/attention3.h"
#include "kernels/attention4.h"
#include "kernels/attention5.h"
#include "kernels/attention6.h"
#include "kernels/attention7.h"
#include "kernels/attention_pool.h"

using namespace xc;
using namespace xcapi;

namespace {

template <typename T, int NW, int NH = 1>
void launch_attn_fwd(AttnParams p, hipStream_t st) {
    p.chunks = (p.n + NW * 32 - 1) / (NW * 32);
    constexpr int lds = attn_fwd_lds_bytes<T, NW, NH>();
    XC_ALLOW_LDS((attn_fwd_kernel<T, NW, NH>), lds);
    hipLaunchKernelGGL((attn_fwd_kernel<T, NW, NH>), dim3(p.batch * p.heads * p.chunks), dim3(NW * 64), lds, st, p);
}
template <typename T, int NW, int NH = 1>
// ... 55 lines not shown
};
int attn_setup(const char* fn, const AttnCall& c, bool ptrs_aligned, AttnParams& p, AttnRoute& route) {
#define XC_REQ(cond, msg) do { if (!(cond)) return xcapi::fail(fn, msg); } while (0)
    XC_REQ(dtype_ok(c.dtype), "bad dtype");
    XC_REQ(c.batch >= 0 && c.n > 0 && c.heads > 0, "bad shape");
    XC_REQ(c.head_dim == 64 || c.head_dim == 128, "head_dim must be 64 or 128 (narrower / in-between widths are zero-padded by the caller)");
    XC_REQ(ptrs_aligned, "pointers must be 16-byte aligned");
    if (c.batch == 0) return 0;
    memset(&p, 0, sizeof(p));
    p.qkv = c.qkv; p.mask = c.mask;
    p.batch = (int)c.batch; p.n = (int)c.n; p.heads = (int)c.heads; p.scale = c.scale; p.causal = c.causal != 0;
    p.first_round = 2 * xc_num_cus();
    XC_REQ(c.dropout_p >= 0.f && c.dropout_p < 1.f, "dropout_p must lie in [0, 1)");
    p.drop_thresh = drop_thresh(c.dropout_p); p.drop_scale = 1.0f / (1.0f - c.dropout_p); p.drop_seed = c.dropout_seed;
    route = attn_route(c.head_dim, c.dtype, c.n, p.drop_thresh != 0);
    XC_REQ((route != ATTN_WIDE_RESIDENT && route != ATTN_RESIDENT) || c.scale > 0.f,
           "the head-resident kernels take the score maximum before scaling: scale must be positive");
    return 0;
#undef XC_REQ
}

template <typename T>
int launch_attn_pool(const AttnPoolParams& p, int64_t head_dim, bool backward, hipStream_t st) {
    const dim3 grid((unsigned)(((int64_t)p.batch * p.heads + 3) / 4)), block(256);
    if (head_dim == 64) {
        if (backward) hipLaunchKernelGGL((attn_pool_bwd_kernel<T, 64>), grid, block, 0, st, p);
        else hipLaunchKernelGGL((attn_pool_fwd_kernel<T, 64>), grid, block, 0, st, p);
    } else {
        if (backward) hipLaunchKernelGGL((attn_pool_bwd_kernel<T, 128>), grid, block, 0, st, p);
        else hipLaunchKernelGGL((attn_pool_fwd_kernel<T, 128>), grid, block, 0, st, p);
    }
    return 0;
}
}

extern "C" {

int xclip_attention_fwd(const void* qkv, const uint8_t* mask, void* out, float* lse, int64_t batch, int64_t n, int64_t heads,
                        int64_t head_dim, float scale, int causal, float dropout_p, uint64_t dropout_seed, int dtype, void* stream) {
    const AttnCall call{qkv, mask, batch, n, heads, head_dim, scale, causal, dropout_p, dropout_seed, dtype};
    AttnParams p; AttnRoute route;
    const int rc = attn_setup(__func__, call, aligned16(qkv) && aligned16(out), p, route);
    if (rc != 0 || batch == 0) return rc;
    p.out = out; p.lse = lse;
    hipStream_t st = (hipStream_t)stream;
    const dim3 hgrid((unsigned)(batch * heads));
    const int nw = attn_waves(n);
    switch (route) {
    case ATTN_WIDE_RESIDENT: {
        const int nwq = a4_fwd_waves((int)n);
        XC_REQUIRE(attn4_fwd_lds_bytes((int)n) <= 160 * 1024, "internal: wide-head forward LDS");
        by_causal(causal, [&](auto c) {
            XC_ALLOW_LDS(attn4_fwd_kernel<decltype(c)::value>, 160 * 1024);
            hipLaunchKernelGGL(attn4_fwd_kernel<decltype(c)::value>, hgrid, dim3(nwq * 64), attn4_fwd_lds_bytes((int)n), st, p);
        });
        break;
    }
    case ATTN_WIDE_TILED:
        by_dtype(dtype, [&](auto t) { by_waves(nw, [&](auto w) { launch_attn_fwd<typename decltype(t)::type, decltype(w)::value, 2>(p, st); }); });
        break;
    case ATTN_RESIDENT: {
        const int nwq = a3_waves((int)n);
        static const int stag = measure_env("XCLIP_ATTN_STAGGER_FWD", -1);
        const int half_head = (int)(1300.0 * (double)n * (double)n / (257.0 * 257.0));
        p.stagger_10ns = (attn3_fwd_lds_bytes((int)n) <= 80 * 1024 && batch * heads >= 1024) ? (stag >= 0 ? stag : half_head) : 0;
        static const int abl_f = measure_env("XCLIP_ATTN_ABL", 0);
        p.chunks = abl_f;
        by_causal(causal, [&](auto c) {
            XC_ALLOW_LDS(attn3_fwd_kernel<decltype(c)::value>, 160 * 1024);
            hipLaunchKernelGGL(attn3_fwd_kernel<decltype(c)::value>, hgrid, dim3(nwq * 64), attn3_fwd_lds_bytes((int)n), st, p);
        });
        break;
    }
    case ATTN_TILED_BF16:
        by_waves(nw, [&](auto w) { launch_attn2_fwd<decltype(w)::value>(p, st); });
        break;
    case ATTN_TILED:
        by_dtype(dtype, [&](auto t) { by_waves(nw, [&](auto w) { launch_attn_fwd<typename decltype(t)::type, decltype(w)::value>(p, st); }); });
        break;
    }
    return check_launch(__func__);
}

int xclip_attention_bwd(const void* qkv, const uint8_t* mask, const void* out, const void* dout, const float* lse,
                        float* delta_ws, void* dqkv, int64_t batch, int64_t n, int64_t heads, int64_t head_dim, float scale, int causal,
                        float dropout_p, uint64_t dropout_seed, int dtype, void* stream) {
    const AttnCall call{qkv, mask, batch, n, heads, head_dim, scale, causal, dropout_p, dropout_seed, dtype};
    AttnParams p; AttnRoute route;
    const int rc = attn_setup(__func__, call, aligned16(qkv) && aligned16(out) && aligned16(dout) && aligned16(dqkv), p, route);
    if (rc != 0 || batch == 0) return rc;
    p.out = const_cast<void*>(out); p.lse = const_cast<float*>(lse); p.dout = dout; p.delta = delta_ws; p.dqkv = dqkv;
    hipStream_t st = (hipStream_t)stream;
    const dim3 hgrid((unsigned)(batch * heads));
    const dim3 dgrid((unsigned)((batch * n + 3) / 4)), dblock(256);
    const int nw = attn_waves(n);
    switch (route) {
    case ATTN_WIDE_RESIDENT: {
        const int nwq = a3_bwd_waves((int)n);
        by_causal(causal, [&](auto c) {
            XC_ALLOW_LDS(attn4_bwd_kernel<decltype(c)::value>, 160 * 1024);
            hipLaunchKernelGGL(attn4_bwd_kernel<decltype(c)::value>, hgrid, dim3(nwq * 64), attn4_bwd_lds_bytes((int)n), st, p);
        });
        break;
    }
    case ATTN_WIDE_TILED:
        XC_REQUIRE(delta_ws != nullptr, "wide heads need the [batch, heads, n] fp32 delta workspace");
        if (dtype == XCLIP_BF16)
            hipLaunchKernelGGL((attn_delta_kernel<bf16_t, 2>), dgrid, dblock, 0, st, (const bf16_t*)out, (const bf16_t*)dout, delta_ws, (int)batch, (int)n, (int)heads);
        else
            hipLaunchKernelGGL((attn_delta_kernel<float, 2>), dgrid, dblock, 0, st, (const float*)out, (const float*)dout, delta_ws, (int)batch, (int)n, (int)heads);
        by_dtype(dtype, [&](auto t) { by_waves(nw, [&](auto w) { launch_attn_bwd<typename decltype(t)::type, decltype(w)::value, 2>(p, st); }); });
        break;
    case ATTN_RESIDENT: {
        static const int bwd_gen = measure_env("XCLIP_ATTN_BWD", 5), min5 = measure_env("XCLIP_ATTN5_MIN", A5_MIN_BLOCKS);
        if (bwd_gen == 6 && a6_takes((int)n, causal)) {
            XC_ALLOW_LDS(attn6_bwd_kernel, 160 * 1024);
            const int64_t heads_total = batch * heads;
            const int cus = xc_num_cus();
            int64_t g6 = heads_total < cus ? heads_total : cus;
            static const int abl6 = measure_env("XCLIP_ATTN6_ABL", 0);
            p.chunks = abl6;
            if (g6 >= 8) g6 &= ~(int64_t)7;
            hipLaunchKernelGGL(attn6_bwd_kernel, dim3((unsigned)g6), dim3(512), A6_LDS_BYTES, st, p);
            return check_launch(__func__);
        }
        if (bwd_gen == 7 && a5_takes((int)n, causal) && (n >> 5) >= min5 && attn5_bwd_lds_bytes((int)n) <= 160 * 1024) {
            XC_ALLOW_LDS(attn7_bwd_kernel, 160 * 1024);
            const int64_t heads_total = batch * heads;
            const int cus = xc_num_cus();
            int64_t g7 = heads_total < cus ? heads_total : cus;
            if (g7 >= 8) g7 &= ~(int64_t)7;
            static const int abl7 = measure_env("XCLIP_ATTN7_ABL", 0);
            p.chunks = abl7;
            hipLaunchKernelGGL(attn7_bwd_kernel, dim3((unsigned)g7), dim3((unsigned)((n >> 5) * 64)), attn5_bwd_lds_bytes((int)n), st, p);
            return check_launch(__func__);
        }
        if (bwd_gen >= 5 && a5_takes((int)n, causal) && (n >> 5) >= min5 && attn5_bwd_lds_bytes((int)n) <= 160 * 1024) {
            XC_ALLOW_LDS(attn5_bwd_kernel, 160 * 1024);
            static const int var5 = measure_env("XCLIP_ATTN5_VAR", 0);
            p.chunks = var5;
            const int64_t g5 = batch * heads;
            hipLaunchKernelGGL(attn5_bwd_kernel, dim3((unsigned)g5), dim3((unsigned)((n >> 5) * 64)), attn5_bwd_lds_bytes((int)n), st, p);
            return check_launch(__func__);
        }
        const int nwq = a3_bwd_waves((int)n);
        static const int abl = measure_env("XCLIP_ATTN_ABL", 0);
        p.chunks = abl;
        static const int stag = measure_env("XCLIP_ATTN_STAGGER_BWD", 0);
        p.stagger_10ns = (attn3_bwd_lds_bytes((int)n) <= 80 * 1024 && batch * heads >= 1024) ? stag : 0;
        by_causal(causal, [&](auto c) {
            XC_ALLOW_LDS(attn3_bwd_kernel<decltype(c)::value>, 160 * 1024);
            hipLaunchKernelGGL(attn3_bwd_kernel<decltype(c)::value>, hgrid, dim3(nwq * 64), attn3_bwd_lds_bytes((int)n), st, p);
        });
        break;
    }
    case ATTN_TILED_BF16:
    case ATTN_TILED:
        by_dtype(dtype, [&](auto t) { using T = typename decltype(t)::type;
            hipLaunchKernelGGL((attn_delta_kernel<T>), dgrid, dblock, 0, st, (const T*)out, (const T*)dout, delta_ws, (int)batch, (int)n, (int)heads);
        });
        if (route == ATTN_TILED_BF16) by_waves(nw, [&](auto w) { launch_attn2_bwd<decltype(w)::value>(p, st); });
        else by_dtype(dtype, [&](auto t) { by_waves(nw, [&](auto w) { launch_attn_bwd<typename decltype(t)::type, decltype(w)::value>(p, st); }); });
        break;
    }
    return check_launch(__func__);
}

int xclip_attention_pool_fwd(const void* q, const void* kv, const uint8_t* mask, void* out, float* lse, int64_t batch, int64_t n,
                             int64_t heads, int64_t head_dim, float scale, int64_t visible_keys, int dtype, void* stream) {
    XC_REQUIRE(dtype_ok(dtype), "bad dtype");
    XC_REQUIRE(batch >= 0 && n > 0 && heads > 0 && visible_keys >= 1 && visible_keys <= n, "bad shape");
    XC_REQUIRE(head_dim == 64 || head_dim == 128, "head_dim must be 64 or 128 (narrower / in-between widths are zero-padded by the caller)");
    XC_REQUIRE(q && kv && out && lse && aligned16(q) && aligned16(kv) && aligned16(out), "pointers must be non-null and 16-byte aligned");
    if (batch == 0) return 0;
    AttnPoolParams p;
    memset(&p, 0, sizeof(p));
    p.q = q; p.kv = kv; p.mask = mask; p.out = out; p.lse = lse;
    p.batch = (int)batch; p.n = (int)n; p.heads = (int)heads; p.nvis = (int)visible_keys; p.scale = scale;
    by_dtype(dtype, [&](auto t) { launch_attn_pool<typename decltype(t)::type>(p, head_dim, false, (hipStream_t)stream); });
    return check_launch(__func__);
}

int xclip_attention_pool_bwd(const void* q, const void* kv, const uint8_t* mask, const void* out, const void* dout, const float* lse,
                             void* dq, void* dkv, int64_t batch, int64_t n, int64_t heads, int64_t head_dim, float scale,
                             int64_t visible_keys, int dtype, void* stream) {
    XC_REQUIRE(dtype_ok(dtype), "bad dtype");
    XC_REQUIRE(batch >= 0 && n > 0 && heads > 0 && visible_keys >= 1 && visible_keys <= n, "bad shape");
    XC_REQUIRE(head_dim == 64 || head_dim == 128, "head_dim must be 64 or 128 (narrower / in-between widths are zero-padded by the caller)");
    XC_REQUIRE(q && kv && out && dout && lse && dq && dkv, "null pointer");
    XC_REQUIRE(aligned16(q) && aligned16(kv) && aligned16(out) && aligned16(dout) && aligned16(dq) && aligned16(dkv), "pointers must be 16-byte aligned");
    if (batch == 0) return 0;
    AttnPoolParams p;
    memset(&p, 0, sizeof(p));
    p.q = q; p.kv = kv; p.mask = mask; p.out = const_cast<void*>(out); p.lse = const_cast<float*>(lse); p.dout = dout; p.dq = dq; p.dkv = dkv;
    p.batch = (int)batch; p.n = (int)n; p.heads = (int)heads; p.nvis = (int)visible_keys; p.scale = scale;
    by_dtype(dtype, [&](auto t) { launch_attn_pool<typename decltype(t)::type>(p, head_dim, true, (hipStream_t)stream); });
    return check_launch(__func__);
}

}
```

x_clip_amd/functional.py:

```python
from __future__ import annotations

from dataclasses import dataclass
from typing import List, Optional, Sequence

import torch
from torch.autograd.function import once_differentiable

from . import ops

Tensor = torch.Tensor

OVERLAP_WGRAD = True
_wgrad_streams = {}

_grad_sinks: list = []


def add_grad_sink(sink) -> None:
    if sink not in _grad_sinks:
        _grad_sinks.append(sink)


def remove_grad_sink(sink) -> None:
    if sink in _grad_sinks:
        _grad_sinks.remove(sink)


def grad_sinks():
    return tuple(_grad_sinks)


def _grad_out(weight: Optional[Tensor], shape, dtype, device) -> Tensor:
    if weight is not None:
        for sink in _grad_sinks:
            out = sink.claim(weight, shape, dtype)
            if out is not None:
                return out
    return torch.empty(*shape, dtype=dtype, device=device)


class _SideGemm:
    def __init__(self, device):
        self.main = self.side = None
        if OVERLAP_WGRAD and device.type == "cuda":
            self.main = torch.cuda.current_stream(device)
            key = (device, self.main.cuda_stream)
            self.side = _wgrad_streams.get(key)
            if self.side is None:
                self.side = _wgrad_streams[key] = torch.cuda.Stream(device=device)
        self.keep = []
        self.pending = []

    def wgrad(self, dy: Tensor, x: Tensor, N1: int, N2: int, M: int, w: Optional[Tensor] = None) -> Tensor:
        out = _grad_out(w, (N1, N2), dy.dtype, dy.device)
        if self.side is None:
            return ops.gemm(dy, x, N1, N2, M, a_kmajor=True, b_kmajor=True, out=out)
        self.side.wait_stream(self.main)
        with torch.cuda.stream(self.side):
            ops.gemm(dy, x, N1, N2, M, a_kmajor=True, b_kmajor=True, out=out)
        self.keep.append((dy, x))
        return out

    def wgrad_into(self, dy: Tensor, x: Tensor, N1: int, N2: int, M: int, out: Tensor) -> Tensor:
        if self.side is None:
            return ops.gemm(dy, x, N1, N2, M, a_kmajor=True, b_kmajor=True, out=out)
        self.side.wait_stream(self.main)
        with torch.cuda.stream(self.side):
            ops.gemm(dy, x, N1, N2, M, a_kmajor=True, b_kmajor=True, out=out)
        self.keep.append((dy, x))
        return out

    def layer_done(self):
        if self.side is None:
            return
        ev = torch.cuda.Event()
        ev.record(self.side)
        self.pending.append((ev, self.keep))
        self.keep = []
        while len(self.pending) > 1:
            ev0, _ = self.pending.pop(0)
            self.main.wait_event(ev0)

    def join(self):
        if self.side is not None:
            self.main.wait_stream(self.side)
        self.keep, self.pending = [], []


def _draw_seed() -> int:
    return int(torch.randint(0, 1 << 62, (1,), dtype=torch.int64).item())


LAYER_PARAMS = 8


@dataclass(frozen=True)
class StackSpec:
    depth: int
    heads: int
    dim_head: int = 64
    checkpoint: bool = False
    rotary: Optional[Tensor] = None
    causal: bool = False
    attn_dropout: float = 0.0
    ff_dropout: float = 0.0

    def __post_init__(self):
        if not 1 <= self.dim_head <= 128:
            raise NotImplementedError("x_clip_amd attention kernels hold heads of up to 128 dimensions (the reference default is 64)")
        if not (0.0 <= self.attn_dropout < 1.0 and 0.0 <= self.ff_dropout < 1.0):
            raise ValueError("dropout probabilities must lie in [0, 1)")

    @property
    def head_slot(self) -> int:
        return 64 if self.dim_head <= 64 else 128


class _GainGrads:

    def __init__(self, gains: Sequence[Tensor]):
        self.sizes = [g.numel() for g in gains]
        self.dtype = gains[0].dtype
        self.flat = torch.zeros(sum(self.sizes), dtype=torch.float32, device=gains[0].device)
        self.views = list(self.flat.split(self.sizes))

    def finish(self) -> List[Tensor]:
        if self.dtype == torch.float32:
            return self.views
        return list(ops.cast_from_f32(self.flat, self.dtype).split(self.sizes))


def _layer_forward(x: Tensor, B: int, n: int, W: Sequence[Tensor], heads: int, mask: Optional[Tensor], rotary: Optional[Tensor] = None,
                   causal: bool = False, scale: float = 0.125, hs: int = 64, drop=(0.0, 0.0, 0)):
    g_attn, w_qkv, w_out, g_out, g_ff, w_ff1, g_inner, w_ff2 = W
    M, D = x.shape
    inner = heads * hs
    p_attn, p_ff, seed = drop
    h, m1, r1 = ops.layernorm_fwd(x, g_attn)
    qkv = ops.gemm(h, w_qkv, M, 3 * inner, D)
    if rotary is not None:
        ops.rotary_(qkv, n, rotary, head_dim=hs)
    o, lse = ops.attention_fwd(qkv.view(B, n, 3 * inner), mask, heads, scale, causal, hs, p_attn, seed)
    p = ops.gemm(o.view(M, inner), w_out, M, D, inner)
    x1, m2, r2, h2, m3, r3 = ops.layernorm_chain_fwd(p, g_out, x, g_ff)
    u = ops.gemm(h2, w_ff1, M, w_ff1.shape[0], D)
    a, m4, r4 = ops.layernorm_fwd(u, g_inner, geglu=True)
    if p_ff > 0.0:
        ops.dropout(a, p_ff, seed + 1, out=a)
    x2 = ops.gemm(a, w_ff2, M, D, a.shape[1], residual=x1)
    return x2, (x, h, m1, r1, qkv, o, lse, p, m2, r2, x1, h2, m3, r3, u, a, m4, r4)


def _layer_backward(dx2: Tensor, saved, B: int, n: int, W: Sequence[Tensor], heads: int, mask: Optional[Tensor],
                    gain_acc: Sequence[Tensor], need_w: Sequence[bool], sg: "_SideGemm", rotary: Optional[Tensor] = None,
                    causal: bool = False, scale: float = 0.125, hs: int = 64, drop=(0.0, 0.0, 0), x2: Optional[Tensor] = None,
                    rowc: Optional[Tensor] = None, below=None):
    p_attn, p_ff, seed = drop
    g_attn, w_qkv, w_out, g_out, g_ff, w_ff1, g_inner, w_ff2 = W
    dg_attn, dg_out, dg_ff, dg_inner = gain_acc
    x, h, m1, r1, qkv, o, lse, p, m2, r2, x1, h2, m3, r3, u, a, m4, r4 = saved
    M, D = x.shape
    inner = heads * hs
    F2 = w_ff1.shape[0]
    Fh = F2 // 2
    if (x2 is not None or rowc is not None) and p_ff == 0.0 and ops.ffn_dgrad_geglu_ok(M, Fh, D, dx2.dtype):
        du, _ = ops.ffn_dgrad_geglu(dx2, w_ff2, u, g_inner, m4, r4, x2, x1, dg=dg_inner, rowc=rowc)
        d_ff2 = sg.wgrad(dx2, a, D, Fh, M, w_ff2) if need_w[3] else None
    else:
        da = ops.gemm(dx2, w_ff2, M, Fh, D, b_kmajor=True)
        d_ff2 = sg.wgrad(dx2, a, D, Fh, M, w_ff2) if need_w[3] else None
        if p_ff > 0.0:
            ops.dropout(da, p_ff, seed + 1, out=da)
        du, _ = ops.layernorm_bwd(da, u, g_inner, m4, r4, geglu=True, dg=dg_inner)
        del da
    dh2 = ops.gemm(du, w_ff1, M, D, F2, b_kmajor=True)
    d_ff1 = sg.wgrad(du, h2, F2, D, M, w_ff1) if need_w[2] else None
    del du
    dx1, dp = ops.layernorm_chain_bwd(dh2, x1, g_ff, m3, r3, dx2, p, g_out, m2, r2, dg_ff, dg_out)
    del dh2
    do = ops.gemm(dp, w_out, M, inner, D, b_kmajor=True)
    d_out = sg.wgrad(dp, o.view(M, inner), D, inner, M, w_out) if need_w[1] else None
    del dp
    dqkv = ops.attention_bwd(qkv.view(B, n, 3 * inner), mask, o, do.view(B, n, inner), lse, heads, scale, causal, hs, p_attn, seed)
    del do
    if rotary is not None:
        ops.rotary_(dqkv.view(M, 3 * inner), n, rotary, inverse=True, head_dim=hs)
    dh = ops.gemm(dqkv.view(M, 3 * inner), w_qkv, M, D, 3 * inner, b_kmajor=True)
    d_qkv = sg.wgrad(dqkv.view(M, 3 * inner), h, 3 * inner, D, M, w_qkv) if need_w[0] else None
    del dqkv
    dx, _ = ops.layernorm_bwd(dh, x, g_attn, m1, r1, dres=dx1, dg=dg_attn, ffn_stats=below)
    return dx, [d_qkv, d_out, d_ff1, d_ff2]


def _pool_view(t2d: Tensor, B: int, n: int, row: int) -> Tensor:
    Wd = t2d.shape[1]
    return t2d.view(B, n * Wd)[:, row * Wd:(row + 1) * Wd]


def _layer_forward_pooled(x: Tensor, B: int, n: int, W: Sequence[Tensor], heads: int, mask: Optional[Tensor], rotary: Optional[Tensor],
                          causal: bool, scale: float, hs: int, row: int):
    g_attn, w_qkv, w_out, g_out, g_ff, w_ff1, g_inner, w_ff2 = W
    M, D = x.shape
    inner = heads * hs
    h, m1, r1 = ops.layernorm_fwd(x, g_attn)
    xc = torch.empty(B, D, dtype=x.dtype, device=x.device)
    ops.copy_rows(_pool_view(x, B, n, row), xc)
    if rotary is None or row == 0:
        q = ops.gemm(_pool_view(h, B, n, row), w_qkv[:inner], B, inner, D)
        kv = ops.gemm(h, w_qkv[inner:], M, 2 * inner, D)
        if rotary is not None:
            ops.rotary_(kv, n, rotary, head_dim=hs)
        oc, lse = ops.attention_pool_fwd(q, kv.view(B, n, 2 * inner), mask, heads, scale, hs, row + 1 if causal else None)
        qkv, o = (q, kv), oc
    else:
        qkv = ops.gemm(h, w_qkv, M, 3 * inner, D)
        ops.rotary_(qkv, n, rotary, head_dim=hs)
        o, lse = ops.attention_fwd(qkv.view(B, n, 3 * inner), mask, heads, scale, causal, hs, 0.0, 0)
        oc = _pool_view(o.view(M, inner), B, n, row)
    p = ops.gemm(oc, w_out, B, D, inner)
    x1, m2, r2, h2, m3, r3 = ops.layernorm_chain_fwd(p, g_out, xc, g_ff)
    u = ops.gemm(h2, w_ff1, B, w_ff1.shape[0], D)
    a, m4, r4 = ops.layernorm_fwd(u, g_inner, geglu=True)
    x2 = ops.gemm(a, w_ff2, B, D, a.shape[1], residual=x1)
    return x2, (x, h, m1, r1, qkv, o, lse, p, m2, r2, x1, h2, m3, r3, u, a, m4, r4)


def _layer_backward_pooled(dx2: Tensor, saved, B: int, n: int, W: Sequence[Tensor], heads: int, mask: Optional[Tensor],
                           gain_acc: Sequence[Tensor], need_w: Sequence[bool], sg: "_SideGemm", rotary: Optional[Tensor], causal: bool,
                           scale: float, hs: int, row: int):
    g_attn, w_qkv, w_out, g_out, g_ff, w_ff1, g_inner, w_ff2 = W
    dg_attn, dg_out, dg_ff, dg_inner = gain_acc
    x, h, m1, r1, qkv, o, lse, p, m2, r2, x1, h2, m3, r3, u, a, m4, r4 = saved
    M, D = x.shape
    inner = heads * hs
    F2 = w_ff1.shape[0]
    Fh = F2 // 2
    da = ops.gemm(dx2, w_ff2, B, Fh, D, b_kmajor=True)
    d_ff2 = sg.wgrad(dx2, a, D, Fh, B, w_ff2) if need_w[3] else None
    du, _ = ops.layernorm_bwd(da, u, g_inner, m4, r4, geglu=True, dg=dg_inner)
    dh2 = ops.gemm(du, w_ff1, B, D, F2, b_kmajor=True)
    d_ff1 = sg.wgrad(du, h2, F2, D, B, w_ff1) if need_w[2] else None
    dx1, dp = ops.layernorm_chain_bwd(dh2, x1, g_ff, m3, r3, dx2, p, g_out, m2, r2, dg_ff, dg_out)
    if rotary is None or row == 0:
        q, kv = qkv
        d_out = sg.wgrad(dp, o, D, inner, B, w_out) if need_w[1] else None
        doc = ops.gemm(dp, w_out, B, inner, D, b_kmajor=True)
        dq, dkv = ops.attention_pool_bwd(q, kv.view(B, n, 2 * inner), mask, o, doc, lse, heads, scale, hs, row + 1 if causal else None)
        if rotary is not None:
            ops.rotary_(dkv.view(M, 2 * inner), n, rotary, inverse=True, head_dim=hs)
        dh = ops.gemm(dkv.view(M, 2 * inner), w_qkv[inner:], M, D, 2 * inner, b_kmajor=True)
        dhq = ops.gemm(dq, w_qkv[:inner], B, D, inner, b_kmajor=True)
        hr = _pool_view(dh, B, n, row)
        t = torch.empty(B, D, dtype=dh.dtype, device=dh.device)
        ops.copy_rows(hr, t)
        ops.copy_rows(ops.add_rows(t, dhq), hr)
        d_qkv = None
        if need_w[0]:
            d_qkv = _grad_out(w_qkv, (3 * inner, D), dp.dtype, dp.device)
            sg.wgrad_into(dq, _pool_view(h, B, n, row), inner, D, B, d_qkv[:inner])
            sg.wgrad_into(dkv.view(M, 2 * inner), h, 2 * inner, D, M, d_qkv[inner:])
        del dkv
    else:
        oc = _pool_view(o.view(M, inner), B, n, row)
        d_out = sg.wgrad(dp, oc, D, inner, B, w_out) if need_w[1] else None
        do = torch.zeros(M, inner, dtype=dp.dtype, device=dp.device)
        ops.gemm(dp, w_out, B, inner, D, b_kmajor=True, out=_pool_view(do, B, n, row))
# ... 467 lines not shown
```

x_clip_amd/ops.py:

```python
from __future__ import annotations

from typing import Optional, Tuple

import math

import torch

from . import _lib

Tensor = torch.Tensor

_DTYPES = {torch.float32: 0, torch.bfloat16: 1}
_U64 = (1 << 64) - 1


def dtype_code(t: Tensor) -> int:
    try:
        return _DTYPES[t.dtype]
    except KeyError:
        raise TypeError(f"x_clip_amd kernels support float32 and bfloat16, got {t.dtype}") from None


def vec(dtype) -> int:
    return 8 if dtype == torch.bfloat16 else 4
# ... 410 lines not shown
        self.under_load_every = under_load_every
        self.record = record
        self._clock = None
        self._clock_n = 0
        self._seen = 0
        self._side = None

    def __enter__(self):
        KernelProbe.active = self
        return self

    def __exit__(self, *exc):
        KernelProbe.active = None

    def _sample(self, t: Tensor, stream, ticks: int):
        if self._clock is None:
            self._clock = torch.zeros(self.clock_slots, 2, dtype=torch.int64, device=t.device)
        if self._clock_n < self.clock_slots:
            _lib.check(_lib.lib().xclip_clock_sample(self._clock[self._clock_n].data_ptr(), ticks, stream.cuda_stream), "xclip_clock_sample")
            self._clock_n += 1

    def begin(self, t: Tensor, family: str = ""):
        if self.under_load_every and family == "gemm":
            self._seen += 1
            if self._seen % self.under_load_every == 0:
                if self._side is None:
                    self._side = torch.cuda.Stream(device=t.device)
                    self._clock = torch.zeros(self.clock_slots, 2, dtype=torch.int64, device=t.device)
                self._side.wait_event(torch.cuda.current_stream(t.device).record_event())
                self._sample(t, self._side, 20000)
        if not self.record:
            return None
        ev0 = torch.cuda.Event(enable_timing=True)
        ev0.record(torch.cuda.current_stream(t.device))
        return ev0

    def end(self, t: Tensor, ev0, family: str, flops: float, nbytes: float, key=None):
        if not self.record:
            return
        ev1 = torch.cuda.Event(enable_timing=True)
        st = torch.cuda.current_stream(t.device)
        ev1.record(st)
        self.records.append((family, flops, ev0, ev1, nbytes, key))
        if self.clock_every and len(self.records) % self.clock_every == 0:
            self._sample(t, st, 1000)

    def summary(self, family: str = "gemm"):
        torch.cuda.synchronize()
        recs = [r for r in self.records if r[0] == family]
        flops = sum(r[1] for r in recs)
        secs = sum(r[2].elapsed_time(r[3]) for r in recs) * 1e-3
        self.algorithmic_bytes = sum(r[4] for r in recs)
        return len(recs), flops, secs

    def by_shape(self):
        torch.cuda.synchronize()
        out = {}
        for r in self.records:
            if r[0] != "gemm":
                continue
            e = out.setdefault(r[5], [0, 0.0])
            e[0] += 1
            e[1] += r[2].elapsed_time(r[3])
        return out

    def clock_mhz(self):
        if self._clock is None or self._clock_n == 0:
            return []
        torch.cuda.synchronize()
        c = self._clock[:self._clock_n].cpu()
        return sorted(float(cy) / max(float(tk), 1.0) * 100.0 for cy, tk in c.tolist() if tk > 0)


GemmProbe = KernelProbe


def _probe(t: Tensor):
    p = KernelProbe.active
    return p if (p is not None and t.is_cuda) else None


def gemm(a: Tensor, b: Tensor, M: int, N: int, K: int, a_kmajor: bool = False, b_kmajor: bool = False, alpha: float = 1.0,
         bias: Optional[Tensor] = None, residual: Optional[Tensor] = None, addrows: Optional[Tensor] = None,
         rowidx: Optional[Tensor] = None, out: Optional[Tensor] = None) -> Tensor:
    _dev_check(a, b, bias, residual, addrows, rowidx, out)
    assert a.dim() == 2 and b.dim() == 2 and a.stride(1) == 1 and b.stride(1) == 1 and a.dtype == b.dtype
    assert tuple(a.shape) == ((K, M) if a_kmajor else (M, K)), (a.shape, M, K, a_kmajor)
    assert tuple(b.shape) == ((K, N) if b_kmajor else (N, K)), (b.shape, N, K, b_kmajor)
    if out is None:
        out = torch.empty(M, N, dtype=a.dtype, device=a.device)
    assert out.dim() == 2 and out.stride(1) == 1 and tuple(out.shape) == (M, N)
    if residual is not None:
        assert residual.dim() == 2 and residual.stride(1) == 1 and tuple(residual.shape) == (M, N)
    if addrows is not None:
        assert rowidx is not None and rowidx.dtype == torch.int32 and rowidx.numel() == M and rowidx.is_contiguous()
        assert addrows.stride(1) == 1 and addrows.shape[1] == N
    L = _lib.lib()
    code = dtype_code(a)
    wbytes = L.xclip_gemm_workspace_bytes(M, N, K, code) if (bias is None and addrows is None and not (BATCH_INVARIANT_GEMM and not a_kmajor)) else 0
    ws = workspace(a.device, wbytes)
    probe = _probe(a)
    ev0 = probe.begin(a, "gemm") if probe is not None else None
    _lib.check(L.xclip_gemm(int(a_kmajor), int(b_kmajor), a.data_ptr(), a.stride(0), b.data_ptr(), b.stride(0), out.data_ptr(),
                            out.stride(0), M, N, K, alpha, _ptr(bias), _ptr(residual),
                            0 if residual is None else residual.stride(0), _ptr(addrows), _ptr(rowidx),
                            0 if addrows is None else addrows.stride(0), _ptr(ws), 0 if ws is None else ws.numel(), code,
                            _stream(a)), "xclip_gemm")
    if probe is not None:
        esz = a.element_size()
        probe.end(a, ev0, "gemm", 2.0 * M * N * K, (M * K + N * K + M * N) * esz + (M * N * esz if residual is not None else 0),
                  (M, N, K, ("T" if a_kmajor else "N") + ("N" if b_kmajor else "T"), residual is not None))
    return out


def gemm_small_limit(max_flop: int = -1) -> int:
    return int(_lib.lib().xclip_gemm_small_limit(int(max_flop)))


def bmm(a: Tensor, b: Tensor, M: int, N: int, K: int, a_kmajor: bool = False, b_kmajor: bool = False, alpha: float = 1.0) -> Tensor:
    _dev_check(a, b)
    assert a.dim() == 3 and b.dim() == 3 and a.shape[0] == b.shape[0] and a.dtype == b.dtype and a.stride(2) == 1 and b.stride(2) == 1
    assert N % vec(a.dtype) == 0
    B = a.shape[0]
    out = torch.empty(B, M, N, dtype=a.dtype, device=a.device)
    for z0 in range(0, B, 65535):
        z1 = min(B, z0 + 65535)
        _lib.check(_lib.lib().xclip_gemm_batched(int(a_kmajor), int(b_kmajor), a[z0:].data_ptr(), a.stride(1), a.stride(0), b[z0:].data_ptr(),
                                                 b.stride(1), b.stride(0), out[z0:].data_ptr(), N, M * N, z1 - z0, M, N, K, alpha,
                                                 dtype_code(a), _stream(a)), "xclip_gemm_batched")
    return out


def rowdot(a: Tensor, b: Tensor) -> Tensor:
    _dev_check(a, b)
    assert a.shape == b.shape and a.dim() == 2 and a.dtype == b.dtype
    v = vec(a.dtype)
    a, b = (t if (t.stride(1) == 1 and t.stride(0) % v == 0 and t.data_ptr() % 16 == 0) else t.contiguous() for t in (a, b))
    out = torch.empty(a.shape[0], dtype=a.dtype, device=a.device)
    _lib.check(_lib.lib().xclip_rowdot(a.data_ptr(), a.stride(0), b.data_ptr(), b.stride(0), out.data_ptr(), a.shape[0], a.shape[1],
                                       dtype_code(a), _stream(a)), "xclip_rowdot")
    return out


def attention_fwd(qkv: Tensor, mask: Optional[Tensor], heads: int, scale: float, causal: bool = False,
                  head_dim: int = 64, dropout_p: float = 0.0, dropout_seed: int = 0) -> Tuple[Tensor, Tensor]:
    _dev_check(qkv, mask)
    qkv = _c(qkv)
    b, n, w = qkv.shape
    assert head_dim in (64, 128) and w == 3 * heads * head_dim, "x_clip_amd attention kernels hold head slots of 64 or 128 features"
    out = torch.empty(b, n, heads * head_dim, dtype=qkv.dtype, device=qkv.device)
    lse = torch.empty(b, heads, n, dtype=torch.float32, device=qkv.device)
    if mask is not None:
        assert mask.dtype == torch.bool and tuple(mask.shape) == (b, n)
        mask = _c(mask)
    probe = _probe(qkv)
    ev0 = probe.begin(qkv) if probe is not None else None
    _lib.check(_lib.lib().xclip_attention_fwd(qkv.data_ptr(), _ptr(mask), out.data_ptr(), lse.data_ptr(), b, n, heads, head_dim, scale,
                                              int(causal), float(dropout_p), int(dropout_seed) & _U64, dtype_code(qkv), _stream(qkv)),
               "xclip_attention_fwd")
    if probe is not None:
        probe.end(qkv, ev0, "attention", 4.0 * b * heads * n * n * head_dim, 4 * b * n * heads * head_dim * qkv.element_size() + 4 * b * heads * n, "attn_fwd")
    return out, lse


def attention_bwd(qkv: Tensor, mask: Optional[Tensor], out: Tensor, dout: Tensor, lse: Tensor, heads: int, scale: float,
                  causal: bool = False, head_dim: int = 64, dropout_p: float = 0.0, dropout_seed: int = 0) -> Tensor:
    _dev_check(qkv, mask, out, dout)
    dout = _c(dout)
    b, n, _ = qkv.shape
    dqkv = torch.empty_like(qkv)
    delta = torch.empty(b, heads, n, dtype=torch.float32, device=qkv.device)
    probe = _probe(qkv)
    ev0 = probe.begin(qkv) if probe is not None else None
    _lib.check(_lib.lib().xclip_attention_bwd(qkv.data_ptr(), _ptr(mask), out.data_ptr(), dout.data_ptr(), lse.data_ptr(),
                                              delta.data_ptr(), dqkv.data_ptr(), b, n, heads, head_dim, scale, int(causal), float(dropout_p),
                                              int(dropout_seed) & _U64, dtype_code(qkv), _stream(qkv)), "xclip_attention_bwd")
    if probe is not None:
        probe.end(qkv, ev0, "attention", 8.0 * b * heads * n * n * head_dim, 8 * b * n * heads * head_dim * qkv.element_size() + 8 * b * heads * n, "attn_bwd")
    return dqkv


def attention_pool_fwd(q: Tensor, kv: Tensor, mask: Optional[Tensor], heads: int, scale: float, head_dim: int = 64,
                       visible_keys: Optional[int] = None) -> Tuple[Tensor, Tensor]:
    _dev_check(q, kv, mask)
    q, kv = _c(q), _c(kv)
    b, n, w = kv.shape
    assert head_dim in (64, 128) and w == 2 * heads * head_dim and tuple(q.shape) == (b, heads * head_dim) and q.dtype == kv.dtype
    out = torch.empty_like(q)
    lse = torch.empty(b, heads, dtype=torch.float32, device=q.device)
    if mask is not None:
        assert mask.dtype == torch.bool and tuple(mask.shape) == (b, n)
        mask = _c(mask)
    probe = _probe(q)
    ev0 = probe.begin(q) if probe is not None else None
    _lib.check(_lib.lib().xclip_attention_pool_fwd(q.data_ptr(), kv.data_ptr(), _ptr(mask), out.data_ptr(), lse.data_ptr(), b, n, heads, head_dim,
                                                   scale, n if visible_keys is None else int(visible_keys), dtype_code(q), _stream(q)),
               "xclip_attention_pool_fwd")
    if probe is not None:
        probe.end(q, ev0, "attention", 4.0 * b * heads * n * head_dim, (2 * b * n + 2 * b) * heads * head_dim * q.element_size(), "attn_pool_fwd")
    return out, lse


def attention_pool_bwd(q: Tensor, kv: Tensor, mask: Optional[Tensor], out: Tensor, dout: Tensor, lse: Tensor, heads: int, scale: float,
                       head_dim: int = 64, visible_keys: Optional[int] = None) -> Tuple[Tensor, Tensor]:
    _dev_check(q, kv, mask, out, dout, lse)
    q, kv, out, dout = _c(q), _c(kv), _c(out), _c(dout)
    b, n, _ = kv.shape
    assert lse.dtype == torch.float32 and lse.is_contiguous() and out.shape == q.shape and dout.shape == q.shape and dout.dtype == q.dtype
    dq = torch.empty_like(q)
    dkv = torch.empty_like(kv)
    probe = _probe(q)
    ev0 = probe.begin(q) if probe is not None else None
    _lib.check(_lib.lib().xclip_attention_pool_bwd(q.data_ptr(), kv.data_ptr(), _ptr(None if mask is None else _c(mask)), out.data_ptr(),
                                                   dout.data_ptr(), lse.data_ptr(), dq.data_ptr(), dkv.data_ptr(), b, n, heads, head_dim, scale,
                                                   n if visible_keys is None else int(visible_keys), dtype_code(q), _stream(q)),
               "xclip_attention_pool_bwd")
    if probe is not None:
        probe.end(q, ev0, "attention", 8.0 * b * heads * n * head_dim, (4 * b * n + 4 * b) * heads * head_dim * q.element_size(), "attn_pool_bwd")
    return dq, dkv


def dropout(x: Tensor, p: float, seed: int, out: Optional[Tensor] = None) -> Tensor:
    _dev_check(x, out)
    assert x.is_contiguous()
    y = torch.empty_like(x) if out is None else out
    _lib.check(_lib.lib().xclip_dropout(x.data_ptr(), y.data_ptr(), x.numel(), float(p), int(seed) & _U64, dtype_code(x), _stream(x)), "xclip_dropout")
    return y


def _scale_args(scale, log_scale: Optional[Tensor]):
    if log_scale is not None:
        assert log_scale.dtype == torch.float32 and log_scale.numel() == 1
    return float(scale), _ptr(log_scale)


def simloss_fwd(q: Tensor, k: Tensor, scale: float, diag_off: int, dcl: bool, coef: float, loss_accum: Optional[Tensor],
                log_scale: Optional[Tensor] = None):
    return simloss_chunked_fwd(q, [(k, 0)], scale, diag_off, dcl, coef, loss_accum, log_scale)


def _chunked_head(q: Tensor, k_chunks, before_chunk, per_slot: int, partial, combine, label: str, neutral=None, stage=None,
                  extra_bytes: int = 0):
    nq, d = q.shape
    slots = sum((kc.shape[0] + 63) // 64 for kc, _ in k_chunks)
    if neutral is not None and (nq == 0 or slots == 0):
        for c in range(len(k_chunks) if before_chunk is not None else 0):
            before_chunk(c)
        return neutral()
    ws = workspace(q.device, per_slot * slots * nq * 4)
    slot0 = 0
    for c, (kc, col0) in enumerate(k_chunks):
        if before_chunk is not None:
            before_chunk(c)
        kc = _c(kc)
        nk = kc.shape[0]
        assert kc.shape[1] == d and kc.dtype == q.dtype
        if nk == 0 and neutral is not None:
            continue
        for kc, col0, s0 in ([(kc, col0, slot0)] if stage is None else stage(kc, col0, slot0)):
            probe = _probe(q)
            ev0 = probe.begin(q) if probe is not None else None
            partial(kc, col0, s0, slots, ws)
# ... 540 lines not shown
```

Baseline: 17980 pairs/s.

## Fuse attention-backward delta rowdot into the output-projection dgrad GEMM epilogue

The dgrad GEMM producing dO (dp @ W_out) now computes, in its epilogue, the per-head dot product of dO with the saved attention output O, and writes it as a float delta tensor. The attention backward kernels take this precomputed delta instead of re-reading O and dO to compute it in their prologue. This removes an extra pass over O and dO in attention backward. In exchange the GEMM epilogue has to stage and read the O tile, which adds LDS traffic, and the delta now comes from bf16-rounded dO values.

```diff
diff --git a/include/xclip.h b/include/xclip.h
--- a/include/xclip.h
+++ b/include/xclip.h
@@ -7,7 +7,7 @@
 #endif
 
 enum { XCLIP_F32 = 0, XCLIP_BF16 = 1 };
-#define XCLIP_ABI_VERSION 28
+#define XCLIP_ABI_VERSION 29
 
 int xclip_abi_version(void);
 const char* xclip_last_error(void);
@@ -66,6 +66,10 @@
                int64_t M, int64_t N, int64_t K, float alpha, const void* bias, const void* residual, int64_t ldr,
                const void* addrows, const int32_t* rowidx, int64_t ld_add, void* workspace, int64_t workspace_bytes,
                int dtype, void* stream);
+int xclip_gemm_rowdot_fused(int64_t M, int64_t N, int64_t K, int b_kmajor, int dtype);
+int xclip_gemm_rowdot(int b_kmajor, const void* A, int64_t lda, const void* B, int64_t ldb, void* C, int64_t ldc, int64_t M, int64_t N,
+                      int64_t K, const void* Y, int64_t ldy, float* rowdot, int64_t group, void* workspace, int64_t workspace_bytes,
+                      int dtype, void* stream);
 int64_t xclip_gemm_small_limit(int64_t max_flop);
 
 int xclip_gemm_batched(int a_kmajor, int b_kmajor, const void* A, int64_t lda, int64_t stride_a, const void* B, int64_t ldb, int64_t stride_b,
@@ -94,6 +98,10 @@
 int xclip_attention_bwd(const void* qkv, const uint8_t* mask, const void* out, const void* dout, const float* lse,
                         float* delta_ws, void* dqkv, int64_t batch, int64_t n, int64_t heads, int64_t head_dim, float scale, int causal,
                         float dropout_p, uint64_t dropout_seed, int dtype, void* stream);
+int xclip_attention_bwd_takes_delta(int64_t n, int64_t head_dim, int causal, float dropout_p, int dtype);
+int xclip_attention_bwd_delta(const void* qkv, const uint8_t* mask, const void* out, const void* dout, const float* lse, const float* delta,
+                              float* delta_ws, void* dqkv, int64_t batch, int64_t n, int64_t heads, int64_t head_dim, float scale, int causal,
+                              float dropout_p, uint64_t dropout_seed, int dtype, void* stream);
 int xclip_attention_pool_fwd(const void* q, const void* kv, const uint8_t* mask, void* out, float* lse, int64_t batch, int64_t n,
                              int64_t heads, int64_t head_dim, float scale, int64_t visible_keys, int dtype, void* stream);
 int xclip_attention_pool_bwd(const void* q, const void* kv, const uint8_t* mask, const void* out, const void* dout, const float* lse,
diff --git a/x_clip_amd/_lib.py b/x_clip_amd/_lib.py
--- a/x_clip_amd/_lib.py
+++ b/x_clip_amd/_lib.py
@@ -40,6 +40,8 @@
     "xclip_gemm_workspace_bytes": (c_int64, [L, L, L, I]),
     "xclip_gemm_small_limit": (c_int64, [L]),
     "xclip_gemm": (c_int, [I, I, P, L, P, L, P, L, L, L, L, F, P, P, L, P, P, L, P, L, I, P]),
+    "xclip_gemm_rowdot_fused": (c_int, [L, L, L, I, I]),
+    "xclip_gemm_rowdot": (c_int, [I, P, L, P, L, P, L, L, L, L, P, L, P, L, P, L, I, P]),
     "xclip_ffn_dgrad_geglu_ok": (c_int, [L, L, L, I]),
     "xclip_ffn_dgrad_geglu_workspace_bytes": (c_int64, [L, L, L]),
     "xclip_ffn_dgrad_geglu": (c_int, [P, L, P, L, P, L, P, P, P, P, L, P, L, P, L, P, P, L, L, L, L, I, P]),
@@ -50,6 +52,8 @@
     "xclip_rowdot": (c_int, [P, L, P, L, P, L, L, I, P]),
     "xclip_attention_fwd": (c_int, [P, P, P, P, L, L, L, L, F, I, F, U, I, P]),
     "xclip_attention_bwd": (c_int, [P, P, P, P, P, P, P, L, L, L, L, F, I, F, U, I, P]),
+    "xclip_attention_bwd_takes_delta": (c_int, [L, L, I, F, I]),
+    "xclip_attention_bwd_delta": (c_int, [P, P, P, P, P, P, P, P, L, L, L, L, F, I, F, U, I, P]),
     "xclip_attention_pool_fwd": (c_int, [P, P, P, P, P, L, L, L, L, F, L, I, P]),
     "xclip_attention_pool_bwd": (c_int, [P, P, P, P, P, P, P, P, L, L, L, L, F, L, I, P]),
     "xclip_dropout": (c_int, [P, P, L, F, U, I, P]),
@@ -98,7 +102,7 @@
     "xclip_adamw_step": (c_int, [P, L, L, I, I, P, P, P, P, P, D, D, D, D, D, P]),
 }
 EXPORTS = tuple(_SIGNATURES)
-ABI_VERSION = 28
+ABI_VERSION = 29
 
 
 def _bind(path: str):
diff --git a/x_clip_amd/csrc/kernels/attention.h b/x_clip_amd/csrc/kernels/attention.h
--- a/x_clip_amd/csrc/kernels/attention.h
+++ b/x_clip_amd/csrc/kernels/attention.h
@@ -23,6 +23,7 @@
     uint32_t drop_thresh;
     float drop_scale;
     uint64_t drop_seed;
+    const float* delta_in;
 };
 
 template <typename T>
diff --git a/x_clip_amd/csrc/kernels/attention3.h b/x_clip_amd/csrc/kernels/attention3.h
--- a/x_clip_amd/csrc/kernels/attention3.h
+++ b/x_clip_amd/csrc/kernels/attention3.h
@@ -438,20 +438,25 @@
     const int nblk = a3_waves(n);
     const int nsub = npad >> 5;
     const float scale2 = p.scale * 1.4426950408889634f;
+    const float* const delta_h = p.delta_in != nullptr ? p.delta_in + ((long)bi * p.heads + hh) * n : nullptr;
     for (int blk = wave; blk < nsub; blk += nwaves) {
         const int row_ = blk * 32 + c31;
         const int rl = row_ < n ? row_ : n - 1;
         const float lse_r = p.lse[((long)bi * p.heads + hh) * n + rl];
         float acc = 0.f;
-#pragma unroll
-        for (int c = 0; c < 4; ++c) {
-            float a[8], b[8];
-            load_vec<bf16_t>(Ob + (long)rl * ldo + h * 32 + c * 8, a);
-            load_vec<bf16_t>(dOb + (long)rl * ldo + h * 32 + c * 8, b);
-#pragma unroll
-            for (int k = 0; k < 8; ++k) acc += a[k] * b[k];
-        }
-        acc += shfl_xor(acc, 32);
+        if (delta_h != nullptr) {
+            acc = delta_h[rl];
+        } else {
+#pragma unroll
+            for (int c = 0; c < 4; ++c) {
+                float a[8], b[8];
+                load_vec<bf16_t>(Ob + (long)rl * ldo + h * 32 + c * 8, a);
+                load_vec<bf16_t>(dOb + (long)rl * ldo + h * 32 + c * 8, b);
+#pragma unroll
+                for (int k = 0; k < 8; ++k) acc += a[k] * b[k];
+            }
+            acc += shfl_xor(acc, 32);
+        }
         if (h == 0) {
             Ds[row_] = row_ < n ? acc : 0.f;
             Ls[row_] = row_ < n ? lse_r * 1.4426950408889634f : 0.f;
diff --git a/x_clip_amd/csrc/kernels/attention5.h b/x_clip_amd/csrc/kernels/attention5.h
--- a/x_clip_amd/csrc/kernels/attention5.h
+++ b/x_clip_amd/csrc/kernels/attention5.h
@@ -168,7 +168,23 @@
         }
         return lse_h[rl];
     };
-    {
+    if (p.delta_in != nullptr) {
+        const float* const delta_h = p.delta_in + ((long)bi * p.heads + hh) * n;
+        auto given = [&](int row_) {
+            const int rl = row_ < n ? row_ : n - 1;
+            const float d = delta_h[rl], l = lse_h[rl];
+            if (h == 0) {
+                Ds[row_] = row_ < n ? d : 0.f;
+                Ls[row_] = row_ < n ? l * 1.4426950408889634f : 0.f;
+            }
+        };
+        a3_dma_image(Qs, Qb, ldq, n, npad, wave, nwaves, lane);
+        a3_dma_image(dOs, dOb, ldo, n, npad, wave, nwaves, lane);
+        a3_dma_image(Ks, Kb, ldq, n, npad, wave, nwaves, lane);
+        a3_key_validity(Ms, p.mask, (long)bi * n, n, npad);
+        given(row);
+        for (int blk = wave + nwaves; blk < nsub; blk += nwaves) given(blk * 32 + c31);
+    } else {
         u32x4 a[4], b[4];
         float lse_r = 0.f;
         if (!(var & 2)) lse_r = delta_rows(row, a, b);
diff --git a/x_clip_amd/csrc/kernels/gemm2.h b/x_clip_amd/csrc/kernels/gemm2.h
--- a/x_clip_amd/csrc/kernels/gemm2.h
+++ b/x_clip_amd/csrc/kernels/gemm2.h
@@ -86,6 +86,8 @@
     int band_n;
     int stream_out;
     int split_lin = 0;
+    float* rowdot = nullptr;
+    int rd_n = 1;
 };
 
 XC_DEV void g2_pair(const Gemm2Params& p, int ntiles, int& tile, int& slice, bool& valid) {
diff --git a/x_clip_amd/csrc/kernels/gemm4.h b/x_clip_amd/csrc/kernels/gemm4.h
--- a/x_clip_amd/csrc/kernels/gemm4.h
+++ b/x_clip_amd/csrc/kernels/gemm4.h
@@ -8,7 +8,8 @@
     G4_PLAIN = 0,
     G4_SLAB = 1,
     G4_TERMS = 2,
-    G4_RES = 3
+    G4_RES = 3,
+    G4_ROWDOT = 4
 };
 
 template <bool KMAJOR>
@@ -603,6 +604,90 @@
             }
         }
     }
+    XC_DEV void rowdot_store(float d, int row, int slot) const {
+        const int b = row / p.rd_n, i = row - b * p.rd_n;
+        p.rowdot[((long)b * (p.N >> 6) + slot) * p.rd_n + i] = d;
+    }
+    static XC_DEV float rowdot_quad(const u32x2 v, const u32x2 y) {
+        return u2f(v[0] << 16) * u2f(y[0] << 16) + u2f(v[0] & 0xffff0000u) * u2f(y[0] & 0xffff0000u) +
+               u2f(v[1] << 16) * u2f(y[1] << 16) + u2f(v[1] & 0xffff0000u) * u2f(y[1] & 0xffff0000u);
+    }
+    XC_DEV void store_full_rowdot_lds(f32x16 (&acc)[4][2], int m0, int n0, unsigned char* scratch) const {
+        const int lane = threadIdx.x & 63, r = lane & 31, h = lane >> 5;
+        const int wave = uniform(threadIdx.x >> 6), wm = wave >> 2, wn = wave & 3;
+        const BufRsrc rc = make_rsrc(p.C + (long)m0 * p.ldc + n0, 255u * (uint32_t)p.ldc * 2u + 512u);
+        const BufRsrc rr = make_rsrc(p.residual + (long)m0 * p.ldr + n0, 255u * (uint32_t)p.ldr * 2u + 512u);
+        const uint32_t vc = ((uint32_t)(wm * 128 + (lane >> 3)) * (uint32_t)p.ldc + (uint32_t)(wn * 64 + 8 * (lane & 7))) * 2u;
+        const uint32_t vr = ((uint32_t)(wm * 128 + (lane >> 3)) * (uint32_t)p.ldr + (uint32_t)(wn * 64 + 8 * (lane & 7))) * 2u;
+        const uint32_t c8 = (uint32_t)p.ldc * 16u, r8 = (uint32_t)p.ldr * 16u;
+        unsigned char* const quad = scratch + r * 128 + 8 * h;
+        unsigned char* const line = scratch + (lane >> 3) * 128 + (((lane & 7) ^ (lane >> 3)) << 4);
+        const float al = p.alpha;
+        const int slot = (n0 >> 6) + wn;
+        u32x4 res[2][4];
+#pragma unroll
+        for (int k = 0; k < 4; ++k) res[0][k] = buf_ld16<0>(rr, vr, r8 * (uint32_t)k);
+#pragma unroll
+        for (int i = 0; i < 4; ++i) {
+            if (i < 3) {
+#pragma unroll
+                for (int k = 0; k < 4; ++k) res[(i + 1) & 1][k] = buf_ld16<0>(rr, vr, r8 * (uint32_t)(4 * (i + 1) + k));
+            }
+#pragma unroll
+            for (int k = 0; k < 4; ++k) *reinterpret_cast<u32x4*>(line + k * 1024) = res[i & 1][k];
+            lds_fence();
+            float d = 0.f;
+#pragma unroll
+            for (int j = 0; j < 2; ++j) {
+#pragma unroll
+                for (int q = 0; q < 4; ++q) {
+                    unsigned char* const at = quad + (((4 * j + q) ^ (r & 7)) << 4);
+                    const u32x2 yv = *reinterpret_cast<const u32x2*>(at);
+                    const float* a = reinterpret_cast<const float*>(&acc[i][j]) + 4 * q;
+                    const u32x2 v = {f2bf_pk(a[0] * al, a[1] * al), f2bf_pk(a[2] * al, a[3] * al)};
+                    d += rowdot_quad(v, yv);
+                    *reinterpret_cast<u32x2*>(at) = v;
+                }
+            }
+            lds_fence();
+            u32x4 o[4];
+#pragma unroll
+            for (int k = 0; k < 4; ++k) o[k] = *reinterpret_cast<const u32x4*>(line + k * 1024);
+            lds_fence();
+#pragma unroll
+            for (int k = 0; k < 4; ++k) buf_st16<0>(rc, vc, c8 * (uint32_t)(4 * i + k), o[k]);
+            d += shfl_xor(d, 32);
+            if (h == 0) rowdot_store(d, m0 + wm * 128 + 32 * i + r, slot);
+        }
+    }
+    XC_DEV void store_ragged_rowdot(f32x16 (&acc)[4][2], int m0, int n0) const {
+        const int lane = threadIdx.x & 63, r = lane & 31, h = lane >> 5;
+        const int wave = uniform(threadIdx.x >> 6), wm = wave >> 2, wn = wave & 3;
+        const int cb = n0 + wn * 64;
+        const float al = p.alpha;
+        if (cb < p.N) {
+#pragma unroll
+            for (int i = 0; i < 4; ++i) {
+                const int row = m0 + wm * 128 + 32 * i + r;
+                const bool valid = row < p.M;
+                const bf16_t* const y = p.residual + (long)(valid ? row : 0) * p.ldr + cb + 4 * h;
+                float d = 0.f;
+#pragma unroll
+                for (int j = 0; j < 2; ++j) {
+#pragma unroll
+                    for (int q = 0; q < 4; ++q) {
+                        const u32x2 yv = valid ? *reinterpret_cast<const u32x2*>(y + 32 * j + 8 * q) : u32x2{0u, 0u};
+                        const float* a = reinterpret_cast<const float*>(&acc[i][j]) + 4 * q;
+                        const u32x2 v = {f2bf_pk(a[0] * al, a[1] * al), f2bf_pk(a[2] * al, a[3] * al)};
+                        d += rowdot_quad(v, yv);
+                    }
+                }
+                d += shfl_xor(d, 32);
+                if (h == 0 && valid) rowdot_store(d, row, cb >> 6);
+            }
+        }
+        store_bf16<false>(acc, m0, n0);
+    }
     XC_DEV void store_full_slab_lds(f32x16 (&acc)[4][2], int m0, int n0, unsigned char* scratch) const {
         const int lane = threadIdx.x & 63, r = lane & 31, h = lane >> 5;
         const int wave = uniform(threadIdx.x >> 6), wm = wave >> 2, wn = wave & 3;
@@ -644,6 +729,10 @@
             store_full_res_lds<false>(acc, m0, n0, scratch);
             return 0;
         }
+        if (MODE == G4_ROWDOT && full) {
+            store_full_rowdot_lds(acc, m0, n0, scratch);
+            return 0;
+        }
         return (*this)(acc, m0, n0);
     }
 
@@ -652,6 +741,10 @@
         if (MODE == G4_PLAIN) {
             if (full) { store_bf16<true>(acc, m0, n0); return 16; }
             store_bf16<false>(acc, m0, n0);
+            return 0;
+        }
+        if (MODE == G4_ROWDOT) {
+            store_ragged_rowdot(acc, m0, n0);
             return 0;
         }
         (void)G3GemmEpilogue<0>{p}(acc, m0, n0);
diff --git a/x_clip_amd/csrc/kernels/rows.h b/x_clip_amd/csrc/kernels/rows.h
--- a/x_clip_amd/csrc/kernels/rows.h
+++ b/x_clip_amd/csrc/kernels/rows.h
@@ -677,4 +677,26 @@
     }
 }
 
-}
+template <typename T>
+__global__ __launch_bounds__(256) void slot_rowdot_kernel(const T* C, long ldc, const T* Y, long ldy, float* out, long M, int slots, int group) {
+    const long id = (long)blockIdx.x * 256 + threadIdx.x;
+    if (id >= M * slots) return;
+    const long m = id / slots;
+    const int s = (int)(id - m * slots);
+    const T* c = C + m * ldc + s * 64;
+    const T* y = Y + m * ldy + s * 64;
+    constexpr int V = Elem<T>::VEC;
+    float acc = 0.f;
+#pragma unroll
+    for (int j = 0; j < 64 / V; ++j) {
+        float a[V], b[V];
+        load_vec<T>(c + j * V, a);
+        load_vec<T>(y + j * V, b);
+#pragma unroll
+        for (int k = 0; k < V; ++k) acc += a[k] * b[k];
+    }
+    const long b_ = m / group;
+    out[(b_ * slots + s) * group + (m - b_ * group)] = acc;
+}
+
+}
diff --git a/x_clip_amd/csrc/xclip_api.hip b/x_clip_amd/csrc/xclip_api.hip
--- a/x_clip_amd/csrc/xclip_api.hip
+++ b/x_clip_amd/csrc/xclip_api.hip
@@ -1033,6 +1033,54 @@
     return check_launch(__func__);
 }
 
+static bool gemm_rowdot_fused(int64_t M, int64_t N, int64_t K, int64_t lda, int64_t ldb, int64_t ldc, int64_t ldy, int dtype) {
+    if (dtype != XCLIP_BF16 || !use_gemm2(M, N, K, dtype) || N % 64 != 0) return false;
+    if (!(lda < (1L << 22) && ldb < (1L << 22) && ldc < (1L << 22) && ldy < (1L << 22) && N < (1L << 21))) return false;
+    GemmArgs g{}; g.M = M; g.N = N; g.K = K; g.lda = lda; g.ldb = ldb;
+    const GemmPlan plan = gemm_plan(g, dtype, INT64_MAX, g_small_flop);
+    return plan.route == GEMM_SMALL || (plan.route == GEMM_256 && plan.splits == 1);
+}
+int xclip_gemm_rowdot_fused(int64_t M, int64_t N, int64_t K, int b_kmajor, int dtype) {
+    return gemm_rowdot_fused(M, N, K, K, b_kmajor ? N : K, N, N, dtype) ? 1 : 0;
+}
+int xclip_gemm_rowdot(int b_kmajor, const void* A, int64_t lda, const void* B, int64_t ldb, void* C, int64_t ldc, int64_t M, int64_t N,
+                      int64_t K, const void* Y, int64_t ldy, float* rowdot, int64_t group, void* workspace, int64_t workspace_bytes,
+                      int dtype, void* stream) {
+    XC_REQUIRE(dtype_ok(dtype), "bad dtype");
+    const int vec = vec_of(dtype);
+    XC_REQUIRE(M >= 0 && N > 0 && K > 0 && group > 0, "bad shape");
+    XC_REQUIRE(N % 64 == 0 && M % group == 0, "N must be a multiple of the 64-column slot and M of the row group");
+    XC_REQUIRE(Y != nullptr && rowdot != nullptr && aligned16(Y) && ldy % vec == 0 && ldy >= N, "Y must be an aligned [M, N] operand");
+    hipStream_t st = (hipStream_t)stream;
+    if (M > 0 && gemm_rowdot_fused(M, N, K, lda, ldb, ldc, ldy, dtype)) {
+        XC_REQUIRE(lda % vec == 0 && ldb % vec == 0 && ldc % vec == 0 && lda >= K && (b_kmajor ? ldb >= N : ldb >= K) && ldc >= N, "bad leading dimensions");
+        XC_REQUIRE(aligned16(A) && aligned16(B) && aligned16(C), "pointers must be 16-byte aligned");
+        Gemm2Params q;
+        q.A = (const bf16_t*)A; q.B = (const bf16_t*)B; q.C = (bf16_t*)C; q.lda = lda; q.ldb = ldb; q.ldc = ldc;
+        q.M = (int)M; q.N = (int)N; q.K = (int)K; q.alpha = 1.f;
+        q.bias = nullptr; q.residual = (const bf16_t*)Y; q.ldr = ldy; q.addrows = nullptr; q.rowidx = nullptr; q.ld_add = 0;
+        q.tiles_m = (int)((M + G2_BM - 1) / G2_BM); q.tiles_n = (int)((N + G2_BN - 1) / G2_BN);
+        q.stream_out = 0; q.band_n = 0; q.k_per_split = (int)K; q.partial = nullptr;
+        q.rowdot = rowdot; q.rd_n = (int)group;
+        int gx = q.tiles_m * q.tiles_n;
+        const int cus = xc_num_cus();
+        if (gx > cus) gx = cus;
+        const dim3 pgrid((unsigned)gx, 1);
+        if (b_kmajor) launch_gemm4<false, true, G4_ROWDOT>(q, pgrid, true, st);
+        else launch_gemm4<false, false, G4_ROWDOT>(q, pgrid, true, st);
+        return check_launch(__func__);
+    }
+    if (const int rc = xclip_gemm(0, b_kmajor, A, lda, B, ldb, C, ldc, M, N, K, 1.f, nullptr, nullptr, 0, nullptr, nullptr, 0, workspace, workspace_bytes,
+                                  dtype, stream)) return rc;
+    if (M == 0) return 0;
+    const int slots = (int)(N / 64);
+    const unsigned blocks = (unsigned)((M * slots + 255) / 256);
+    by_dtype(dtype, [&](auto t) { using T = typename decltype(t)::type;
+        hipLaunchKernelGGL((slot_rowdot_kernel<T>), dim3(blocks), dim3(256), 0, st, (const T*)C, (long)ldc, (const T*)Y, (long)ldy, rowdot, (long)M, slots, (int)group);
+    });
+    return check_launch(__func__);
+}
+
 int xclip_ffn_dgrad_geglu_ok(int64_t M, int64_t F, int64_t D, int dtype) {
     return dtype == XCLIP_BF16 && M > 0 && M % G2_BM == 0 && F % G2_BN == 0 && D % G2_BK == 0 && D >= 2 * G2_BK && D <= 4096 && F < (1L << 20) &&
            (M / G2_BM) * (F / G2_BN) < (1L << 30);
diff --git a/x_clip_amd/csrc/xclip_attn.hip b/x_clip_amd/csrc/xclip_attn.hip
--- a/x_clip_amd/csrc/xclip_attn.hip
+++ b/x_clip_amd/csrc/xclip_attn.hip
@@ -161,9 +161,23 @@
     return check_launch(__func__);
 }
 
+inline bool attn_bwd_takes_delta(AttnRoute route, int causal) { return route == ATTN_RESIDENT && !causal; }
+
+int xclip_attention_bwd_takes_delta(int64_t n, int64_t head_dim, int causal, float dropout_p, int dtype) {
+    if (!dtype_ok(dtype) || n <= 0 || (head_dim != 64 && head_dim != 128) || !(dropout_p >= 0.f && dropout_p < 1.f)) return 0;
+    return attn_bwd_takes_delta(attn_route(head_dim, dtype, n, drop_thresh(dropout_p) != 0), causal) ? 1 : 0;
+}
+
 int xclip_attention_bwd(const void* qkv, const uint8_t* mask, const void* out, const void* dout, const float* lse,
                         float* delta_ws, void* dqkv, int64_t batch, int64_t n, int64_t heads, int64_t head_dim, float scale, int causal,
                         float dropout_p, uint64_t dropout_seed, int dtype, void* stream) {
+    return xclip_attention_bwd_delta(qkv, mask, out, dout, lse, nullptr, delta_ws, dqkv, batch, n, heads, head_dim, scale, causal, dropout_p,
+                                     dropout_seed, dtype, stream);
+}
+
+int xclip_attention_bwd_delta(const void* qkv, const uint8_t* mask, const void* out, const void* dout, const float* lse, const float* delta,
+                              float* delta_ws, void* dqkv, int64_t batch, int64_t n, int64_t heads, int64_t head_dim, float scale, int causal,
+                              float dropout_p, uint64_t dropout_seed, int dtype, void* stream) {
     const AttnCall call{qkv, mask, batch, n, heads, head_dim, scale, causal, dropout_p, dropout_seed, dtype};
     AttnParams p; AttnRoute route;
     const int rc = attn_setup(__func__, call, aligned16(qkv) && aligned16(out) && aligned16(dout) && aligned16(dqkv), p, route);
@@ -214,6 +228,7 @@
             hipLaunchKernelGGL(attn7_bwd_kernel, dim3((unsigned)g7), dim3((unsigned)((n >> 5) * 64)), attn5_bwd_lds_bytes((int)n), st, p);
             return check_launch(__func__);
         }
+        if (attn_bwd_takes_delta(route, causal)) p.delta_in = delta;
         if (bwd_gen >= 5 && a5_takes((int)n, causal) && (n >> 5) >= min5 && attn5_bwd_lds_bytes((int)n) <= 160 * 1024) {
             XC_ALLOW_LDS(attn5_bwd_kernel, 160 * 1024);
             static const int var5 = measure_env("XCLIP_ATTN5_VAR", 0);
diff --git a/x_clip_amd/functional.py b/x_clip_amd/functional.py
--- a/x_clip_amd/functional.py
+++ b/x_clip_amd/functional.py
@@ -90,6 +90,8 @@
 def _draw_seed() -> int:
     return int(torch.randint(0, 1 << 62, (1,), dtype=torch.int64).item())
 
+
+USE_ATTN_DELTA = True
 
 LAYER_PARAMS = 8
 
@@ -178,10 +180,14 @@
     del du
     dx1, dp = ops.layernorm_chain_bwd(dh2, x1, g_ff, m3, r3, dx2, p, g_out, m2, r2, dg_ff, dg_out)
     del dh2
-    do = ops.gemm(dp, w_out, M, inner, D, b_kmajor=True)
+    delta = None
+    if USE_ATTN_DELTA and ops.gemm_rowdot_ok(M, inner, hs, n) and ops.attention_bwd_takes_delta(n, hs, causal, p_attn, dp.dtype):
+        do, delta = ops.gemm(dp, w_out, M, inner, D, b_kmajor=True, rowdot=(o.view(M, inner), hs, n))
+    else:
+        do = ops.gemm(dp, w_out, M, inner, D, b_kmajor=True)
     d_out = sg.wgrad(dp, o.view(M, inner), D, inner, M, w_out) if need_w[1] else None
     del dp
-    dqkv = ops.attention_bwd(qkv.view(B, n, 3 * inner), mask, o, do.view(B, n, inner), lse, heads, scale, causal, hs, p_attn, seed)
+    dqkv = ops.attention_bwd(qkv.view(B, n, 3 * inner), mask, o, do.view(B, n, inner), lse, heads, scale, causal, hs, p_attn, seed, delta=delta)
     del do
     if rotary is not None:
         ops.rotary_(dqkv.view(M, 3 * inner), n, rotary, inverse=True, head_dim=hs)
diff --git a/x_clip_amd/ops.py b/x_clip_amd/ops.py
--- a/x_clip_amd/ops.py
+++ b/x_clip_amd/ops.py
@@ -516,7 +516,10 @@
 
 def gemm(a: Tensor, b: Tensor, M: int, N: int, K: int, a_kmajor: bool = False, b_kmajor: bool = False, alpha: float = 1.0,
          bias: Optional[Tensor] = None, residual: Optional[Tensor] = None, addrows: Optional[Tensor] = None,
-         rowidx: Optional[Tensor] = None, out: Optional[Tensor] = None) -> Tensor:
+         rowidx: Optional[Tensor] = None, out: Optional[Tensor] = None, rowdot=None):
+    if rowdot is not None:
+        assert alpha == 1.0 and not a_kmajor and bias is None and residual is None and addrows is None
+        return _gemm_rowdot(a, b, M, N, K, b_kmajor, out, *rowdot)
     _dev_check(a, b, bias, residual, addrows, rowidx, out)
     assert a.dim() == 2 and b.dim() == 2 and a.stride(1) == 1 and b.stride(1) == 1 and a.dtype == b.dtype
     assert tuple(a.shape) == ((K, M) if a_kmajor else (M, K)), (a.shape, M, K, a_kmajor)
@@ -545,6 +548,41 @@
         probe.end(a, ev0, "gemm", 2.0 * M * N * K, (M * K + N * K + M * N) * esz + (M * N * esz if residual is not None else 0),
                   (M, N, K, ("T" if a_kmajor else "N") + ("N" if b_kmajor else "T"), residual is not None))
     return out
+
+
+def gemm_rowdot_ok(M: int, N: int, slot: int, group: int) -> bool:
+    return slot == 64 and N % 64 == 0 and group > 0 and M % group == 0
+
+
+def gemm_rowdot_fused(M: int, N: int, K: int, b_kmajor: bool, dtype) -> bool:
+    return bool(_lib.lib().xclip_gemm_rowdot_fused(M, N, K, int(b_kmajor), 1 if dtype == torch.bfloat16 else 0))
+
+
+def _gemm_rowdot(a: Tensor, b: Tensor, M: int, N: int, K: int, b_kmajor: bool, out: Optional[Tensor], y: Tensor, slot: int = 64,
+                 group: Optional[int] = None) -> Tuple[Tensor, Tensor]:
+    group = M if group is None else int(group)
+    assert gemm_rowdot_ok(M, N, slot, group), (M, N, slot, group)
+    _dev_check(a, b, y, out)
+    assert a.dim() == 2 and b.dim() == 2 and a.stride(1) == 1 and b.stride(1) == 1 and a.dtype == b.dtype == y.dtype
+    assert tuple(a.shape) == (M, K) and tuple(b.shape) == ((K, N) if b_kmajor else (N, K))
+    assert y.dim() == 2 and y.stride(1) == 1 and tuple(y.shape) == (M, N)
+    if out is None:
+        out = torch.empty(M, N, dtype=a.dtype, device=a.device)
+    assert out.dim() == 2 and out.stride(1) == 1 and tuple(out.shape) == (M, N)
+    delta = torch.empty(M // group, N // 64, group, dtype=torch.float32, device=a.device)
+    L = _lib.lib()
+    code = dtype_code(a)
+    wbytes = 0 if BATCH_INVARIANT_GEMM else L.xclip_gemm_workspace_bytes(M, N, K, code)
+    ws = workspace(a.device, wbytes)
+    probe = _probe(a)
+    ev0 = probe.begin(a, "gemm") if probe is not None else None
+    _lib.check(L.xclip_gemm_rowdot(int(b_kmajor), a.data_ptr(), a.stride(0), b.data_ptr(), b.stride(0), out.data_ptr(), out.stride(0), M, N, K,
+                                   y.data_ptr(), y.stride(0), delta.data_ptr(), group, _ptr(ws), 0 if ws is None else ws.numel(), code,
+                                   _stream(a)), "xclip_gemm_rowdot")
+    if probe is not None:
+        esz = a.element_size()
+        probe.end(a, ev0, "gemm", 2.0 * M * N * K, (M * K + N * K + 2 * M * N) * esz, (M, N, K, "N" + ("N" if b_kmajor else "T"), False))
+    return out, delta
 
 
 def gemm_small_limit(max_flop: int = -1) -> int:
@@ -598,20 +636,32 @@
 
 
 def attention_bwd(qkv: Tensor, mask: Optional[Tensor], out: Tensor, dout: Tensor, lse: Tensor, heads: int, scale: float,
-                  causal: bool = False, head_dim: int = 64, dropout_p: float = 0.0, dropout_seed: int = 0) -> Tensor:
-    _dev_check(qkv, mask, out, dout)
+                  causal: bool = False, head_dim: int = 64, dropout_p: float = 0.0, dropout_seed: int = 0, delta: Optional[Tensor] = None) -> Tensor:
+    _dev_check(qkv, mask, out, dout, delta)
     dout = _c(dout)
     b, n, _ = qkv.shape
     dqkv = torch.empty_like(qkv)
-    delta = torch.empty(b, heads, n, dtype=torch.float32, device=qkv.device)
     probe = _probe(qkv)
-    ev0 = probe.begin(qkv) if probe is not None else None
-    _lib.check(_lib.lib().xclip_attention_bwd(qkv.data_ptr(), _ptr(mask), out.data_ptr(), dout.data_ptr(), lse.data_ptr(),
-                                              delta.data_ptr(), dqkv.data_ptr(), b, n, heads, head_dim, scale, int(causal), float(dropout_p),
-                                              int(dropout_seed) & _U64, dtype_code(qkv), _stream(qkv)), "xclip_attention_bwd")
+    if delta is not None:
+        assert delta.dtype == torch.float32 and delta.is_contiguous() and tuple(delta.shape) == (b, heads, n)
+        ws = torch.empty(b, heads, n, dtype=torch.float32, device=qkv.device) if not attention_bwd_takes_delta(n, head_dim, causal, dropout_p, qkv.dtype) else None
+        ev0 = probe.begin(qkv) if probe is not None else None
+        _lib.check(_lib.lib().xclip_attention_bwd_delta(qkv.data_ptr(), _ptr(mask), out.data_ptr(), dout.data_ptr(), lse.data_ptr(), delta.data_ptr(),
+                                                        _ptr(ws), dqkv.data_ptr(), b, n, heads, head_dim, scale, int(causal), float(dropout_p),
+                                                        int(dropout_seed) & _U64, dtype_code(qkv), _stream(qkv)), "xclip_attention_bwd_delta")
+    else:
+        ws = torch.empty(b, heads, n, dtype=torch.float32, device=qkv.device)
+        ev0 = probe.begin(qkv) if probe is not None else None
+        _lib.check(_lib.lib().xclip_attention_bwd(qkv.data_ptr(), _ptr(mask), out.data_ptr(), dout.data_ptr(), lse.data_ptr(),
+                                                  ws.data_ptr(), dqkv.data_ptr(), b, n, heads, head_dim, scale, int(causal), float(dropout_p),
+                                                  int(dropout_seed) & _U64, dtype_code(qkv), _stream(qkv)), "xclip_attention_bwd")
     if probe is not None:
         probe.end(qkv, ev0, "attention", 8.0 * b * heads * n * n * head_dim, 8 * b * n * heads * head_dim * qkv.element_size() + 8 * b * heads * n, "attn_bwd")
     return dqkv
+
+
+def attention_bwd_takes_delta(n: int, head_dim: int, causal: bool, dropout_p: float, dtype) -> bool:
+    return bool(_lib.lib().xclip_attention_bwd_takes_delta(n, head_dim, int(causal), float(dropout_p), 1 if dtype == torch.bfloat16 else 0))
 
 
 def attention_pool_fwd(q: Tensor, kv: Tensor, mask: Optional[Tensor], heads: int, scale: float, head_dim: int = 64,
```

New measurement: 18030 pairs/s, median of 6. Within noise of the previous version (+0.3%).
